# oadrian/GPUFluidSimulator

Measured on AMD Instinct MI355X. Metric: particle-steps/sec, higher is better.
Workload: dtype f32; 1 GPU; dam-break C3: 256x256x256 = 16777216 particles, grid 512^3, box 32.0, dt 5e-7, jittered lattice, FLOWING: timed after 6000 run-up steps on the device (+5 warm-up); particles=16777216, parallelism=1 GPU, whole domain, state=flow, runup_steps=6000

## Files before the change

gpufluidsimulator_amd/capi.py:

```python
from __future__ import annotations

import ctypes as C
import os

import numpy as np

HERE = os.path.dirname(os.path.abspath(__file__))
LIB_PATH = os.environ.get("SPH_HIP_LIB", os.path.join(HERE, "libsph_hip.so"))

PHASES = ("z-index", "sort", "b-grid", "dens", "force", "collision", "integrate")
HALO_RECORD_FLOATS = 8


class SphError(RuntimeError):
    pass


EXCHANGE_FN = C.CFUNCTYPE(C.c_int, C.c_void_p, C.c_int, C.c_void_p, C.c_size_t, C.c_void_p, C.c_size_t, C.c_void_p, C.c_size_t,
                          C.c_void_p, C.c_size_t, C.c_void_p)


class Transport(C.Structure):
    _fields_ = [("self", C.c_void_p), ("exchange", EXCHANGE_FN), ("host_buffers", C.c_int),
                ("abort", C.CFUNCTYPE(None, C.c_void_p))]
# ... 130 lines not shown
    "sph_slab_set_protocol": (C.c_int, [_P, C.c_int]),
    "sph_slab_protocol": (C.c_int, [_P, C.POINTER(C.c_uint64)]),
    "sph_destroy": (None, [_P]),
    "sph_set_stream": (C.c_int, [_P, _P]),
    "sph_set_params": (C.c_int, [_P, C.POINTER(Params)]),
    "sph_get_params": (C.c_int, [_P, C.POINTER(Params)]),
    "sph_sync": (C.c_int, [_P]),
    "sph_num_particles": (_U32, [_P]),
    "sph_capacity": (_U32, [_P]),
    "sph_upload": (C.c_int, [_P, _U32, _P, _P, _P]),
    "sph_set_by_index": (C.c_int, [_P, _U32, _U32, C.c_void_p, C.c_void_p]),
    "sph_reset_lattice": (C.c_int, [_P, C.POINTER(_U32), C.c_int, C.POINTER(C.c_float), C.c_uint64, _U32]),
    "sph_download": (C.c_int, [_P, _U32, _U32, _P, _P, _P, _P]),
    "sph_download_owned": (C.c_int, [_P, _P, _P, _P]),
    "sph_download_forces": (C.c_int, [_P, _U32, _U32, _P, _P, _P, _P]),
    "sph_snapshot_save": (C.c_int, [_P, C.c_char_p]),
    "sph_snapshot_load": (C.c_int, [_P, C.c_char_p]),
    "sph_snapshot_info": (C.c_int, [C.c_char_p, C.POINTER(_U32), C.POINTER(Params)]),
    "sph_set_colliders": (C.c_int, [_P, _U32, C.POINTER(Collider)]),
    "sph_get_colliders": (C.c_int, [_P, C.POINTER(_U32), C.POINTER(Collider)]),
    "sph_set_collider_bodies": (C.c_int, [_P, _U32, C.POINTER(ColliderBody)]),
    "sph_get_collider_impulses": (C.c_int, [_P, C.POINTER(_U32), C.POINTER(C.c_double), C.POINTER(C.c_uint64)]),
    "sph_emit": (C.c_int, [_P, _U32, _P, _P, _P, C.POINTER(_U32)]),
    "sph_remove": (C.c_int, [_P, _U32, C.POINTER(Region), C.POINTER(_U32), _P, _U32]),
    "sph_count_in_regions": (C.c_int, [_P, _U32, C.POINTER(Region), C.POINTER(_U32)]),
    "sph_camera_look_at": (C.c_int, [C.POINTER(Camera), _U32, _U32, C.POINTER(C.c_float), C.POINTER(C.c_float),
                                     C.POINTER(C.c_float), C.c_float, C.c_float, C.c_float]),
    "sph_render": (C.c_int, [_P, C.POINTER(Camera), C.POINTER(RenderStyle)]),
    "sph_render_read": (C.c_int, [_P, _P, _P, _P]),
    "sph_render_image_dev": (C.c_int, [_P, C.POINTER(_P), C.POINTER(_U32), C.POINTER(_U32)]),
    "sph_surface_defaults": (None, [C.POINTER(SurfaceStyle)]),
    "sph_render_surface": (C.c_int, [_P, C.POINTER(Camera), C.POINTER(RenderStyle), C.POINTER(SurfaceStyle)]),
    "sph_render_surface_read": (C.c_int, [_P, _P, _P, _P]),
    "sph_obstacle_lattice": (C.c_int, [_P, C.c_float, C.POINTER(C.c_float), C.POINTER(C.c_float), C.POINTER(ObstacleGrid)]),
    "sph_obstacle_build": (C.c_int, [_P, C.c_float, C.POINTER(C.c_float), C.POINTER(C.c_float), _U32, C.POINTER(Shape)]),
    "sph_obstacle_set_grid": (C.c_int, [_P, C.POINTER(ObstacleGrid), _P]),
    "sph_obstacle_clear": (C.c_int, [_P]),
    "sph_obstacle_set_motion": (C.c_int, [_P, C.POINTER(C.c_float), C.POINTER(C.c_float)]),
    "sph_obstacle_get": (C.c_int, [_P, C.POINTER(ObstacleGrid), C.POINTER(C.c_float), C.POINTER(C.c_float)]),
    "sph_obstacle_read": (C.c_int, [_P, _P]),
    "sph_obstacle_sample": (C.c_int, [_P, _U32, _P, _P, _P, _P]),
    "sph_obstacle_build_mesh": (C.c_int, [_P, C.POINTER(ObstacleMeshParams), C.POINTER(C.c_float), C.POINTER(C.c_float), _U32, _P,
                                          _U32, _P]),
    "sph_obstacle_build_mesh_dev": (C.c_int, [_P, C.POINTER(ObstacleMeshParams), C.POINTER(C.c_float), C.POINTER(C.c_float), _U32,
                                              _P, _U32, _P]),
    "sph_obstacle_build_obj": (C.c_int, [_P, C.POINTER(ObstacleMeshParams), C.POINTER(C.c_float), C.POINTER(C.c_float), C.c_char_p]),
    "sph_obstacle_mesh_stats": (C.c_int, [_P, C.POINTER(C.c_uint64)]),
    "sph_mesh_defaults": (None, [C.POINTER(MeshParams)]),
    "sph_mesh_lattice": (C.c_int, [_P, C.POINTER(MeshParams), C.POINTER(_U32), C.POINTER(C.c_float)]),
    "sph_mesh_extract": (C.c_int, [_P, C.POINTER(MeshParams), C.POINTER(_U32), C.POINTER(_U32)]),
    "sph_mesh_read": (C.c_int, [_P, _P, _P, _P]),
    "sph_mesh_dev": (C.c_int, [_P, C.POINTER(_P), C.POINTER(_P), C.POINTER(_P), C.POINTER(_U32), C.POINTER(_U32)]),
    "sph_mesh_save_obj": (C.c_int, [_P, C.c_char_p]),
    "sph_mesh_field_dims": (C.c_int, [_P, C.POINTER(_U32)]),
    "sph_mesh_field_read": (C.c_int, [_P, _P]),
    "sph_positions_dev": (C.c_int, [_P, C.POINTER(_P)]),
    "sph_download_positions4": (C.c_int, [_P, _P]),
    "sph_get_keys": (C.c_int, [_P, _P]),
    "sph_get_order": (C.c_int, [_P, _P]),
    "sph_get_cell_range": (C.c_int, [_P, _U32, C.POINTER(_U32), C.POINTER(_U32)]),
    "sph_get_cells": (C.c_int, [_P, _U32, _P, _P, _P]),
    "sph_cell_key": (_U32, [_P, _U32, _U32, _U32]),
    "sph_hash": (C.c_int, [_P]),
    "sph_sort": (C.c_int, [_P]),
    "sph_build_cells": (C.c_int, [_P]),
    "sph_density": (C.c_int, [_P]),
    "sph_force": (C.c_int, [_P]),
    "sph_collide": (C.c_int, [_P]),
    "sph_integrate": (C.c_int, [_P, C.c_float]),
    "sph_step": (C.c_int, [_P, C.c_float, _U32]),
    "sph_step_phased": (C.c_int, [_P, C.c_float, _U32]),
    "sph_force_collide_integrate": (C.c_int, [_P, C.c_float]),
    "sph_timing_enable": (C.c_int, [_P, C.c_int]),
    "sph_timing_get": (C.c_int, [_P, C.POINTER(C.c_float), C.POINTER(_U32)]),
    "sph_timing_reset": (C.c_int, [_P]),
    "sph_last_sort_skipped": (C.c_int, [_P]),
    "sph_sort_stats": (C.c_int, [_P, C.POINTER(C.c_uint64), C.POINTER(C.c_uint64), C.POINTER(C.c_uint64), C.POINTER(C.c_uint32),
                                 C.POINTER(C.c_uint64)]),
    "sph_set_sort_mode": (C.c_int, [_P, C.c_int]),
    "sph_set_direct_hull": (C.c_int, [_P, C.c_uint32]),
    "sph_set_pair_small_launch": (C.c_int, [_P, C.c_uint32]),
    "sph_set_block_order": (C.c_int, [_P, C.c_int, C.c_int, C.c_uint32]),
    "sph_sort_forms": (C.c_int, [_P, C.POINTER(C.c_uint64)]),
    "sph_test_trust_mover_hint": (C.c_int, [_P]),
    "sph_memory_stats": (None, [C.POINTER(C.c_uint64)]),
    "sph_test_fail_alloc": (None, [C.c_uint32]),
    "sph_test_guard": (None, [C.c_uint32, C.c_int]),
    "sph_test_guard_check": (C.c_int, [C.POINTER(C.c_uint64)]),
    "sph_test_scan": (C.c_int, [_P, C.c_int, C.c_uint32, C.c_void_p, C.c_void_p, C.c_void_p]),
    "sph_test_lower_bounds": (C.c_int, [_P, C.c_void_p, C.c_uint32, C.c_void_p, C.c_uint32, C.c_void_p]),
    "sph_set_precision": (C.c_int, [_P, C.c_int]),
    "sph_get_precision": (C.c_int, [_P]),
    "sph_migrants_count": (C.c_int, [_P, C.POINTER(_U32)]),
    "sph_slab_counts": (C.c_int, [_P, C.POINTER(_U32)]),
    "sph_migrants_pack": (C.c_int, [_P, C.POINTER(_P), _U32]),
    "sph_migrants_append": (C.c_int, [_P, _P, _U32]),
    "sph_halo_count": (C.c_int, [_P, C.POINTER(_U32)]),
    "sph_halo_pack": (C.c_int, [_P, C.POINTER(_P), _U32]),
    "sph_halo_pack_counts": (C.c_int, [_P, C.POINTER(_P), _U32, C.POINTER(_U32)]),
    "sph_halo_unpack": (C.c_int, [_P, _P, _U32, _P, _U32]),
    "sph_halo_pack_density": (C.c_int, [_P, C.POINTER(_P), _U32]),
    "sph_halo_unpack_density": (C.c_int, [_P, _P, _P]),
    "sph_layer_histogram": (C.c_int, [_P, _P, _U32]),
    "sph_rccl_unique_id": (C.c_int, [C.c_void_p]),
    "sph_rccl_transport_create": (C.c_int, [C.POINTER(C.POINTER(Transport)), C.c_void_p, C.c_int, C.c_int, C.c_int]),
    "sph_rccl_transport_destroy": (None, [C.POINTER(Transport)]),
    "sph_rccl_transport_selftest": (C.c_int, [C.POINTER(Transport), C.c_size_t]),
    "sph_rccl_transport_info": (C.c_int, [C.POINTER(Transport), C.POINTER(C.c_int)]),
    "sph_slab_ping": (C.c_int, [_P, C.c_size_t, _U32, C.POINTER(C.c_double)]),
    "sph_slab_recut": (C.c_int, [_P, _U32, _U32]),
    "sph_slab_recut_stats": (C.c_int, [_P, C.POINTER(C.c_uint64)]),
    "sph_slab_set_early_force": (C.c_int, [_P, C.c_int]),
    "sph_slab_early_force_stats": (C.c_int, [_P, C.POINTER(C.c_uint64)]),
    "sph_slab_timing_enable": (C.c_int, [_P, C.c_int]),
    "sph_slab_timing_reset": (C.c_int, [_P]),
    "sph_slab_timing_get": (C.c_int, [_P, C.POINTER(C.c_double)]),
    "sph_slab_test_raise_flag": (C.c_int, [_P, C.c_int]),
    "sph_slab_in_place_merges": (C.c_uint64, [C.c_void_p]),
    "sph_slab_exchanges": (C.c_uint64, [C.c_void_p]),
    "sph_slab_failed": (C.c_int, [C.c_void_p]),
    "sph_slab_create": (C.c_int, [C.POINTER(_P), _P, C.c_int, C.c_int, C.POINTER(Transport), _U32]),
    "sph_slab_destroy": (None, [_P]),
    "sph_slab_step": (C.c_int, [_P, C.c_float, _U32]),
    "sph_slab_sync": (C.c_int, [_P]),
    "sph_slab_stats": (C.c_int, [_P, C.POINTER(C.c_uint64)]),
    "sph_slab_counters": (C.c_int, [_P, C.POINTER(C.c_uint64)]),
    "sph_slab_set_wait_timeout": (C.c_int, [_P, C.c_double]),
    "sph_local_hub_create": (C.c_int, [C.POINTER(_P), C.c_int, C.c_int]),
    "sph_local_hub_destroy": (None, [_P]),
    "sph_local_hub_set_timeout": (C.c_int, [_P, C.c_double]),
    "sph_local_transport_create": (C.c_int, [C.POINTER(C.POINTER(Transport)), _P, C.c_int]),
    "sph_local_transport_destroy": (None, [C.POINTER(Transport)]),
    "sph_loop_transport_create": (C.c_int, [C.POINTER(C.POINTER(Transport)), C.c_float, C.c_double, C.c_double]),
    "sph_loop_transport_destroy": (None, [C.POINTER(Transport)]),
    "sph_ic_dam_break": (None, [C.POINTER(_U32), C.POINTER(C.c_float), C.c_int, C.c_uint64, C.c_uint64, _P, _P]),
    "sph_ic_random_box": (None, [C.c_uint64, C.POINTER(C.c_float), C.c_float, _U32, C.c_float, _P, _P]),
}

_lib = None
_torch_first = None


def load():
    global _lib, _torch_first
    if _lib is None:
        import sys
        _torch_first = "torch" in sys.modules
        if not os.path.exists(LIB_PATH):
            from . import build as _b
            _b.build()
        lib = C.CDLL(LIB_PATH)
        lenient = bool(os.environ.get("SPH_HIP_LIB_ALLOW_MISSING"))
        for name, (res, args) in SIGNATURES.items():
            if lenient and not hasattr(lib, name):
                continue
            fn = getattr(lib, name)
            fn.restype = res
            fn.argtypes = args
        if lib.sph_abi_version() != 2:
            raise SphError("libsph_hip.so ABI version mismatch")
        _lib = lib
    return _lib


def _check(rc):
    if rc < 0:
# ... 423 lines not shown

    def positions_dev(self):
        p = _P()
        _check(self.L.sph_positions_dev(self.h, C.byref(p)))
        return p.value

    def keys(self):
        out = np.empty(self.n, dtype=np.uint32)
        _check(self.L.sph_get_keys(self.h, out.ctypes.data))
        return out

    def order(self):
        out = np.empty(self.n, dtype=np.uint32)
        _check(self.L.sph_get_order(self.h, out.ctypes.data))
        return out

    def cells(self, max_cells=None):
        max_cells = self.n + 16 if max_cells is None else max_cells
        k = np.empty(max_cells, dtype=np.uint32)
        s = np.empty(max_cells, dtype=np.uint32)
        c = np.empty(max_cells, dtype=np.uint32)
        m = _check(self.L.sph_get_cells(self.h, max_cells, k.ctypes.data, s.ctypes.data, c.ctypes.data))
        m = min(m, max_cells)
        return k[:m], s[:m], c[:m]

    def cell_range(self, cell):
        a, b = _U32(), _U32()
        _check(self.L.sph_get_cell_range(self.h, int(cell), C.byref(a), C.byref(b)))
        return a.value, b.value

    def cell_key(self, x, y, z):
        return int(self.L.sph_cell_key(self.h, int(x), int(y), int(z)))

    def hash(self): _check(self.L.sph_hash(self.h))
    def sort(self): _check(self.L.sph_sort(self.h))
    def build_cells(self): _check(self.L.sph_build_cells(self.h))
    def density(self): _check(self.L.sph_density(self.h))
    def force(self): _check(self.L.sph_force(self.h))
    def collide(self): _check(self.L.sph_collide(self.h))
    def integrate(self, dt): _check(self.L.sph_integrate(self.h, float(dt)))
    def step(self, dt, n=1): _check(self.L.sph_step(self.h, float(dt), int(n)))
    def step_phased(self, dt, n=1): _check(self.L.sph_step_phased(self.h, float(dt), int(n)))
    def sync(self): _check(self.L.sph_sync(self.h))

    def timing(self, on=True): _check(self.L.sph_timing_enable(self.h, 1 if on else 0))
    def timing_reset(self): _check(self.L.sph_timing_reset(self.h))

    def sort_skipped(self):
        return bool(self.L.sph_last_sort_skipped(self.h))

    def sort_stats(self):
        a, b, k, m, t = C.c_uint64(), C.c_uint64(), C.c_uint64(), C.c_uint32(), C.c_uint64()
        _check(self.L.sph_sort_stats(self.h, C.byref(a), C.byref(b), C.byref(k), C.byref(m), C.byref(t)))
        return {"sorts": a.value, "merges": b.value, "skips": k.value, "last_movers": m.value, "movers_total": t.value}

    def set_precision(self, mixed_f16=False):
        _check(self.L.sph_set_precision(self.h, 1 if mixed_f16 else 0))

    def set_sort_mode(self, merge=True):
        _check(self.L.sph_set_sort_mode(self.h, int(merge)))

    def trust_mover_hint(self):
        _check(self.L.sph_test_trust_mover_hint(self.h))

    def test_scan(self, values):
        v = np.ascontiguousarray(values)
        assert v.ndim == 1 and v.dtype in (np.uint32, np.uint64), v.dtype
        out, total = np.empty_like(v), np.zeros(1, v.dtype)
        _check(self.L.sph_test_scan(self.h, 8 * v.dtype.itemsize, v.size, v.ctypes.data, out.ctypes.data, total.ctypes.data))
        return out, total[0]

    def test_lower_bounds(self, keys, targets):
        k, t = np.ascontiguousarray(keys), np.ascontiguousarray(targets)
        assert k.ndim == 1 and t.ndim == 1 and k.dtype == np.uint32 and t.dtype == np.uint32, (k.dtype, t.dtype)
        out = np.empty(t.size, np.uint32)
        _check(self.L.sph_test_lower_bounds(self.h, k.ctypes.data, k.size, t.ctypes.data, t.size, out.ctypes.data))
        return out

    def sort_forms(self):
        out = (C.c_uint64 * 3)()
        _check(self.L.sph_sort_forms(self.h, out))
        return tuple(int(v) for v in out)

    def set_block_order(self, xcd=True, ztile=True, strip_blocks_log2=4):
        _check(self.L.sph_set_block_order(self.h, int(bool(xcd)), int(bool(ztile)), int(strip_blocks_log2)))

    def set_direct_hull(self, slots=512):
        _check(self.L.sph_set_direct_hull(self.h, int(slots) & 0xFFFFFFFF))

    def set_pair_small_launch(self, slots):
        _check(self.L.sph_set_pair_small_launch(self.h, int(slots) & 0xFFFFFFFF))

    def timing_get(self):
        ms = (C.c_float * len(PHASES))()
        steps = _U32(0)
        _check(self.L.sph_timing_get(self.h, ms, C.byref(steps)))
        return {PHASES[k]: float(ms[k]) for k in range(len(PHASES))}, int(steps.value)

    def _pair(self, fn, *a):
        cnt = (_U32 * 2)()
        _check(fn(self.h, cnt, *a))
        return int(cnt[0]), int(cnt[1])

    def slab_counts(self):
        cnt = (_U32 * 4)()
        _check(self.L.sph_slab_counts(self.h, cnt))
        return tuple(int(v) for v in cnt)

    def force_collide_integrate(self, dt): _check(self.L.sph_force_collide_integrate(self.h, float(dt)))

    def migrants_count(self): return self._pair(self.L.sph_migrants_count)
    def halo_count(self): return self._pair(self.L.sph_halo_count)

    def migrants_pack(self, buf_lo, buf_hi, capacity):
        _check(self.L.sph_migrants_pack(self.h, (_P * 2)(buf_lo, buf_hi), int(capacity)))

    def migrants_append(self, buf, n):
        _check(self.L.sph_migrants_append(self.h, _P(buf), int(n)))

    def halo_pack(self, buf_lo, buf_hi, capacity, counts=None):
        if counts is None:
            _check(self.L.sph_halo_pack(self.h, (_P * 2)(buf_lo, buf_hi), int(capacity)))
        else:
            _check(self.L.sph_halo_pack_counts(self.h, (_P * 2)(buf_lo, buf_hi), int(capacity),
                                               (_U32 * 2)(int(counts[0]), int(counts[1]))))

    def halo_unpack(self, lo, n_lo, hi, n_hi):
        _check(self.L.sph_halo_unpack(self.h, _P(lo), int(n_lo), _P(hi), int(n_hi)))

    def halo_pack_density(self, buf_lo, buf_hi, capacity):
        _check(self.L.sph_halo_pack_density(self.h, (_P * 2)(buf_lo, buf_hi), int(capacity)))

    def halo_unpack_density(self, lo, hi):
        _check(self.L.sph_halo_unpack_density(self.h, _P(lo), _P(hi)))

    def layer_histogram(self):
        n = int(self.params.grid[2])
        out = np.zeros(n, dtype=np.uint32)
        _check(self.L.sph_layer_histogram(self.h, out.ctypes.data, n))
        return out
```

gpufluidsimulator_amd/csrc/sph_capi.hip:

```cpp
#include "sph_device.hpp"

#include <cmath>
#include <cstdarg>
#include <cstdlib>
#include <cstring>
#include <mutex>
#include <new>
#include <vector>

namespace sph {

template <class T>
__global__ __launch_bounds__(1024) void k_test_scan(const T* __restrict__ in, uint32_t n, T* __restrict__ out, T* __restrict__ total) {
    __shared__ T lds[1024 / 64];
    const T sum = scan_array_one_block<1024>(n, lds, [&](uint32_t i) { return in[i]; }, [&](uint32_t i, T before) { out[i] = before; });
    if (threadIdx.x == 0) *total = sum;
}

template <class T>
static int test_scan(sph_ctx* c, Buffers& mem, uint32_t n, const void* in, void* out, void* total) {
    T *d_in = nullptr, *d_out = nullptr, *d_total = nullptr;
    int rc;
    if ((rc = mem.alloc(&d_in, n, false)) || (rc = mem.alloc(&d_out, n, false)) || (rc = mem.alloc(&d_total, 1, false))) return rc;
    if (n) SPH_HIP(hipMemcpyAsync(d_in, in, (size_t)n * sizeof(T), hipMemcpyHostToDevice, c->stream));
// ... 171 lines not shown
    ph.gas_constant = p->gas_constant;
    const float poly6 = 315.f / (65.f * PI_F * powf(p->h, 9.f));
    const float spiky = 45.f / (PI_F * powf(p->h, 6.f));
    ph.poly6_mass = p->mass * poly6;
    ph.spiky_half_mass = p->mass * spiky * 0.5f;
    const float visc = p->viscosity != 0.f ? p->viscosity : 1.f;
    ph.visc_coef = (visc * p->mass) * spiky;
    ph.cp_scale = ph.spiky_half_mass / ph.visc_coef;
    ph.visc_on = p->viscosity != 0.f ? 1.f : 0.f;
    ph.gravity_y = p->gravity_y;
    ph.wall_eps = p->wall_eps;
    ph.wall_damping = p->wall_damping;
    const double cd = (double)p->collision_param * 2.0 * (double)p->particle_radius;
    float r2max = (float)(cd * cd);
    for (int k = 0; k < 8; k++) r2max = nextafterf(r2max, INFINITY);
    while ((double)sqrtf(r2max) > cd) r2max = nextafterf(r2max, 0.f);
    ph.coll_dist2 = r2max;
    ph.coll_mass = p->mass * (1.f + p->restitution);
    for (int a = 0; a < 3; a++) { ph.box_min[a] = p->box_min[a]; ph.box_max[a] = p->box_max[a]; }
    return SPH_OK;
}

static int create_impl(sph_ctx** out, int device, uint32_t capacity, const sph_params* p, uint32_t z_lo, uint32_t z_hi,
                       uint32_t gcap, bool slab, uint32_t ghost_layers = 1) {
    SPH_REQUIRE(out && p, SPH_E_INVALID, "null argument");
    *out = nullptr;
    SPH_REQUIRE(capacity > 0 && (uint64_t)capacity + 2ull * gcap < (1ull << 31), SPH_E_INVALID, "bad capacity");
    int ndev = 0;
    hipError_t e = hipGetDeviceCount(&ndev);
    if (e != hipSuccess || ndev <= 0) {
        set_error("no HIP device available (%s): libsph_hip has no CPU fallback", hipGetErrorString(e));
        return SPH_E_DEVICE;
    }
    if (device < 0) device = g_device;
    SPH_REQUIRE(device < ndev, SPH_E_DEVICE, "device %d out of range (%d devices)", device, ndev);
    SPH_HIP(hipSetDevice(device));
    hipDeviceProp_t prop;
    SPH_HIP(hipGetDeviceProperties(&prop, device));
    if (strncmp(prop.gcnArchName, "gfx950", 6) != 0) {
        set_error("device %d is %s; libsph_hip is built for gfx950 (MI355X) only", device, prop.gcnArchName);
        return SPH_E_DEVICE;
    }
    sph_ctx* c = new (std::nothrow) sph_ctx();
    SPH_REQUIRE(c, SPH_E_NOMEM, "out of host memory");
    c->device = device;
    c->ghost_layers = slab ? ghost_layers : 1u;
    int rc = derive(c, p, z_lo, z_hi, slab);
    if (rc) { delete c; return rc; }
    c->cap = capacity; c->gcap = gcap; c->tot = capacity + 2 * gcap; c->slab = slab;
    c->own_off = gcap;
    c->pos_out_cap = slab ? 0 : capacity;
    Buffers& m = c->mem;
    const size_t tot = (size_t)c->tot + 256;
    rc = m.alloc(&c->posi, tot, true);
    if (!rc) rc = m.alloc(&c->velr, tot, true);
    if (!rc) rc = m.alloc(&c->posi2, tot, true);
    if (!rc) rc = m.alloc(&c->velr2, tot, true);
    if (!rc) rc = m.alloc(&c->keyS, tot, true);
    if (!rc) rc = m.alloc(&c->keyS2, tot, true);
    if (!rc) rc = m.alloc(&c->dp, tot, true);
    if (!rc) rc = m.alloc(&c->cw, tot, true);
    if (!rc) rc = m.alloc(&c->fpress, tot, false);
    if (!rc) rc = m.alloc(&c->fvisc, tot, false);
    if (!rc) rc = m.alloc(&c->dvel, tot, false);
    if (!rc) rc = m.alloc(&c->pos_out, (size_t)c->pos_out_cap, false);
    if (!rc) rc = m.alloc(&c->table.base, (size_t)c->grid.ncells + 2, true);
    if (!rc) table_init(c, c->table.base, c->grid.ncells);
    if (!rc) rc = sort_buffers_alloc(c);
    if (const char* env = getenv("SPH_BLOCK_ORDER")) {
        int x = 1, z = 1, sh = 4, zd = 1, xr = 1;
        if (sscanf(env, "%d,%d,%d,%d,%d", &x, &z, &sh, &zd, &xr) >= 1) {
            c->order_xcd = x != 0; c->order_ztile = z != 0; if (sh >= 1 && sh <= 10) c->order_strip_sh = (uint32_t)sh;
            c->order_ztile_dens = zd != 0; c->order_xrot = xr != 0;
        }
    }
    if (const char* env = getenv("SPH_PAIR_SMALL_SLOTS")) {
        unsigned long v = 0;
        if (sscanf(env, "%lu", &v) == 1) c->pair_small_slots = v > 0xFFFFFFFFul ? 0xFFFFFFFFu : (uint32_t)v;
    }
    if (const char* env = getenv("SPH_PAIR_CLAMP")) {
        int v = 1;
        if (sscanf(env, "%d", &v) == 1) c->pair_clamp = v != 0;
    }
    if (rc) { m.free_all(); delete c; return rc; }
    *out = c;
    return SPH_OK;
}

void timing_collect(sph_ctx* c) {
    for (size_t k = 0; k + 3 <= c->events.size(); k += 3) {
        hipEvent_t a = c->events[k], b = c->events[k + 1];
        int phase = (int)(intptr_t)c->events[k + 2];
        hipEventSynchronize(b);
        float ms = 0.f;
        if (hipEventElapsedTime(&ms, a, b) == hipSuccess) c->ph_ms[phase] += ms;
        hipEventDestroy(a);
        hipEventDestroy(b);
    }
    c->events.clear();
}

int step_hash(sph_ctx* c, bool ghosts_to_sort) {
    PhaseTimer t(c, SPH_PH_ZINDEX);
    const SlotRange live = live_slots(c);
    int rc = c->sort_merge && c->order_valid && table_covers(c, live.lo, live.hi) ? table_leave_to_sort(c, ghosts_to_sort)
                                                                                 : launch_cells_clear(c);
    if (rc) return rc;
    rc = launch_hash(c);
    if (rc) return rc;
    c->keys_fresh = false;
    c->stage = sph_ctx::ST_HASHED;
    return SPH_OK;
}

int step_sort(sph_ctx* c, bool* owned_build_pending) {
    PhaseTimer t(c, SPH_PH_SORT);
    int rc = launch_sort(c, owned_build_pending);
    if (rc) return rc;
    c->n_glo = c->n_ghi = 0;
    c->halo_n_valid = false;
    c->stage = sph_ctx::ST_SORTED;
    results_stale(c);
    return SPH_OK;
}

int step_cells(sph_ctx* c) {
    PhaseTimer t(c, SPH_PH_BGRID);
    const SlotRange live = live_slots(c);
    if (!table_covers(c, live.lo, live.hi)) {
        int rc = launch_cells_build(c);
        if (rc) return rc;
    }
    c->stage = sph_ctx::ST_CELLS;
    return SPH_OK;
}

static int do_density(sph_ctx* c) {
    PhaseTimer t(c, SPH_PH_DENS);
    int rc = launch_density(c);
    if (rc) return rc;
    c->have_dens = true;
    return SPH_OK;
}

}

namespace sph {
int set_slab_range(sph_ctx* c, uint32_t z_lo, uint32_t z_hi) {
    SPH_REQUIRE(c && c->slab, SPH_E_INVALID, "set_slab_range needs a slab context");
    sph_ctx tmp;
    tmp.params = c->params;
    tmp.ghost_layers = c->ghost_layers;
    int rc = derive(&tmp, &c->params, z_lo, z_hi, true);
    if (rc) return rc;
    if (tmp.grid.ncells > c->table.alloc) {
        SPH_HIP(hipStreamSynchronize(c->stream));
        uint2* base = nullptr;
        rc = c->mem.alloc(&base, (size_t)tmp.grid.ncells + 2, true);
        if (rc) return rc;
        c->mem.release(&c->table.base);
        table_init(c, base, tmp.grid.ncells);
    }
    c->grid = tmp.grid; c->z_lo = z_lo; c->z_hi = z_hi; c->key_bits = tmp.key_bits;
    table_forget(c);
    order_lost(c);
    results_stale(c);
    c->n_glo = c->n_ghi = 0;
    c->halo_n_valid = false;
    return SPH_OK;
}
}

using namespace sph;

__global__ __launch_bounds__(256) void k_set_by_index(float4* __restrict__ posi, float4* __restrict__ velr, uint32_t n,
                                                      uint32_t first, uint32_t count, const float* __restrict__ pos,
                                                      const float* __restrict__ vel, float4* __restrict__ pos_by_index) {
    const uint32_t i = blockIdx.x * 256u + threadIdx.x;
    if (i >= n) return;
    float4 p = posi[i];
    const uint32_t k = __float_as_uint(p.w) - first;
    if (k >= count) return;
    if (pos) {
        p.x = pos[3 * k]; p.y = pos[3 * k + 1]; p.z = pos[3 * k + 2];
        posi[i] = p;
        if (pos_by_index) pos_by_index[first + k] = make_float4(p.x, p.y, p.z, 1.0f);
    }
    if (vel) velr[i] = make_float4(vel[3 * k], vel[3 * k + 1], vel[3 * k + 2], 0.f);
}


__global__ __launch_bounds__(256) void k_gather_cells(const uint32_t* __restrict__ keys, uint32_t m,
                                                      const uint2* __restrict__ cells, uint2* __restrict__ out) {
    const uint32_t k = blockIdx.x * 256u + threadIdx.x;
    if (k < m) out[k] = cells[keys[k]];
}

static inline uint32_t idx_of(const float4& p) { uint32_t u; memcpy(&u, &p.w, 4); return u; }

static int install_records(sph_ctx* c, uint32_t n, const float4* hp, const float4* hv) {
// ... 542 lines not shown
        }
        tmp.free_all();
        if (rc) return rc;
        for (uint32_t k = 0; k < take; k++) {
            if (key) key[k] = uniq[k];
            if (start) start[k] = got[k].x - lo;
            if (count) count[k] = got[k].y - got[k].x;
        }
    }
    return (int)m;
}

uint32_t sph_cell_key(const sph_ctx* c, uint32_t x, uint32_t y, uint32_t z) {
    if (!c) return 0;
    return ((uint32_t)((int32_t)z - c->grid.z_off) * c->grid.g[1] + y) * c->grid.g[0] + x;
}

int sph_hash(sph_ctx* c) {
    SPH_REQUIRE(c, SPH_E_INVALID, "null context");
    SPH_HIP(hipSetDevice(c->device));
    return step_hash(c);
}

int sph_sort(sph_ctx* c) {
    SPH_REQUIRE(c, SPH_E_INVALID, "null context");
    SPH_REQUIRE(c->stage == sph_ctx::ST_HASHED, SPH_E_STATE, "sph_sort needs sph_hash first");
    SPH_HIP(hipSetDevice(c->device));
    return step_sort(c);
}

int sph_build_cells(sph_ctx* c) {
    SPH_REQUIRE(c, SPH_E_INVALID, "null context");
    SPH_REQUIRE(c->stage >= sph_ctx::ST_SORTED, SPH_E_STATE, "sph_build_cells needs sph_sort first");
    SPH_HIP(hipSetDevice(c->device));
    return step_cells(c);
}

int sph_density(sph_ctx* c) {
    SPH_REQUIRE(c, SPH_E_INVALID, "null context");
    SPH_REQUIRE(c->stage >= sph_ctx::ST_CELLS && c->table.valid, SPH_E_STATE, "sph_density needs sph_build_cells first");
    SPH_HIP(hipSetDevice(c->device));
    return do_density(c);
}

int sph_force(sph_ctx* c) {
    SPH_REQUIRE(c, SPH_E_INVALID, "null context");
    SPH_REQUIRE(c->stage >= sph_ctx::ST_CELLS && c->have_dens, SPH_E_STATE, "sph_force needs sph_density first");
    SPH_HIP(hipSetDevice(c->device));
    PhaseTimer t(c, SPH_PH_FORCE);
    int rc = launch_force(c, true, false, false, 0.f);
    if (rc) return rc;
    c->have_force = true;
    return SPH_OK;
}

int sph_collide(sph_ctx* c) {
    SPH_REQUIRE(c, SPH_E_INVALID, "null context");
    SPH_REQUIRE(c->stage >= sph_ctx::ST_CELLS && c->table.valid, SPH_E_STATE, "sph_collide needs sph_build_cells first");
    SPH_HIP(hipSetDevice(c->device));
    PhaseTimer t(c, SPH_PH_COLLISION);
    int rc = launch_force(c, false, true, false, 0.f);
    if (rc) return rc;
    c->have_coll = true;
    return SPH_OK;
}

int sph_integrate(sph_ctx* c, float dt) {
    SPH_REQUIRE(c, SPH_E_INVALID, "null context");
    SPH_REQUIRE(c->have_dens && c->have_force && c->have_coll, SPH_E_STATE,
                "sph_integrate needs sph_density, sph_force and sph_collide first");
    SPH_HIP(hipSetDevice(c->device));
    PhaseTimer t(c, SPH_PH_INTEGRATE);
    int rc = launch_integrate(c, dt);
    if (rc) return rc;
    c->have_force = c->have_coll = false;
    return SPH_OK;
}

int sph_step(sph_ctx* c, float dt, uint32_t n_steps) {
    SPH_REQUIRE(c, SPH_E_INVALID, "null context");
    SPH_HIP(hipSetDevice(c->device));
    for (uint32_t s = 0; s < n_steps; s++) {
        int rc = step_hash(c);
        if (!rc) rc = step_sort(c);
        if (!rc) rc = step_cells(c);
        if (!rc) rc = do_density(c);
        if (rc) return rc;
        {
            PhaseTimer t(c, SPH_PH_FORCE);
            rc = launch_force(c, true, true, true, dt);
            if (rc) return rc;
        }
        c->have_force = c->have_coll = false;
        if (c->timing) { c->timed_steps++; if (c->events.size() > 3 * 4096) timing_collect(c); }
    }
    return SPH_OK;
}

int sph_force_collide_integrate(sph_ctx* c, float dt) {
    SPH_REQUIRE(c, SPH_E_INVALID, "null context");
    SPH_REQUIRE(c->stage >= sph_ctx::ST_CELLS && c->have_dens, SPH_E_STATE,
                "sph_force_collide_integrate needs sph_density first");
    SPH_HIP(hipSetDevice(c->device));
    PhaseTimer t(c, SPH_PH_FORCE);
    int rc = launch_force(c, true, true, true, dt);
    if (rc) return rc;
    c->have_force = c->have_coll = false;
    return SPH_OK;
}

int sph_step_phased(sph_ctx* c, float dt, uint32_t n_steps) {
    for (uint32_t s = 0; s < n_steps; s++) {
        int rc = sph_hash(c);
        if (!rc) rc = sph_sort(c);
        if (!rc) rc = sph_build_cells(c);
        if (!rc) rc = sph_density(c);
        if (!rc) rc = sph_force(c);
        if (!rc) rc = sph_collide(c);
        if (!rc) rc = sph_integrate(c, dt);
        if (rc) return rc;
        if (c->timing) { c->timed_steps++; if (c->events.size() > 3 * 4096) timing_collect(c); }
    }
    return SPH_OK;
}

int sph_timing_enable(sph_ctx* c, int on) {
    SPH_REQUIRE(c, SPH_E_INVALID, "null context");
    c->timing = on != 0;
    return SPH_OK;
}

int sph_timing_get(sph_ctx* c, float ms[SPH_PH_COUNT], uint32_t* n_steps) {
    SPH_REQUIRE(c && ms, SPH_E_INVALID, "null argument");
    SPH_HIP(hipSetDevice(c->device));
    timing_collect(c);
    for (int k = 0; k < SPH_PH_COUNT; k++) ms[k] = (float)c->ph_ms[k];
    if (n_steps) *n_steps = c->timed_steps;
    return SPH_OK;
}

int sph_timing_reset(sph_ctx* c) {
    SPH_REQUIRE(c, SPH_E_INVALID, "null context");
    SPH_HIP(hipSetDevice(c->device));
    timing_collect(c);
    for (int k = 0; k < SPH_PH_COUNT; k++) c->ph_ms[k] = 0;
    c->timed_steps = 0;
    return SPH_OK;
}

int sph_last_sort_skipped(const sph_ctx* c) { return c && c->last_sort_skipped ? 1 : 0; }

int sph_set_precision(sph_ctx* c, int precision) {
    SPH_REQUIRE(c, SPH_E_INVALID, "null context");
    SPH_REQUIRE(precision == SPH_PRECISION_F32 || precision == SPH_PRECISION_MIXED_F16, SPH_E_INVALID,
                "unknown precision %d", precision);
    c->precision = precision;
    return SPH_OK;
}

int sph_get_precision(const sph_ctx* c) { return c ? c->precision : SPH_PRECISION_F32; }

int sph_set_sort_mode(sph_ctx* c, int merge) {
    SPH_REQUIRE(c, SPH_E_INVALID, "null context");
    c->sort_merge = merge != 0;
    c->sort_merge_always = merge == 2;
    return SPH_OK;
}

int sph_test_trust_mover_hint(sph_ctx* c) {
    SPH_REQUIRE(c, SPH_E_INVALID, "null context");
    c->sort_form_both_until = 0;
    return SPH_OK;
}

int sph_sort_forms(const sph_ctx* c, uint64_t out[3]) {
    SPH_REQUIRE(c && out, SPH_E_INVALID, "null argument");
    for (int k = 0; k < 3; k++) out[k] = c->sort_forms[k];
    return SPH_OK;
}

int sph_set_block_order(sph_ctx* c, int xcd, int ztile, uint32_t strip_blocks_log2) {
    SPH_REQUIRE(c, SPH_E_INVALID, "null context");
    SPH_REQUIRE(strip_blocks_log2 >= 1u && strip_blocks_log2 <= 10u, SPH_E_INVALID, "strip of 2^%u blocks", strip_blocks_log2);
    c->order_xcd = xcd != 0;
    c->order_ztile = c->order_ztile_dens = ztile != 0;
    c->order_strip_sh = strip_blocks_log2;
    return SPH_OK;
}

int sph_set_direct_hull(sph_ctx* c, uint32_t slots) {
    SPH_REQUIRE(c, SPH_E_INVALID, "null context");
    c->direct_hull = slots;
    return SPH_OK;
}

int sph_set_pair_small_launch(sph_ctx* c, uint32_t slots) {
    SPH_REQUIRE(c, SPH_E_INVALID, "null context");
    c->pair_small_slots = slots;
    return SPH_OK;
}

int sph_sort_stats(sph_ctx* c, uint64_t* sorts, uint64_t* merges, uint64_t* skips, uint32_t* last_movers,
                   uint64_t* movers_total) {
    SPH_REQUIRE(c, SPH_E_INVALID, "null context");
    SPH_HIP(hipSetDevice(c->device));
    SPH_HIP(hipStreamSynchronize(c->stream));
    if (movers_total) {
        unsigned long long t = 0;
        SPH_HIP(hipMemcpy(&t, c->mm_total, sizeof(t), hipMemcpyDeviceToHost));
        *movers_total = t;
    }
    if (sorts) *sorts = c->sort_calls;
    if (merges) *merges = c->sort_merges;
    if (skips) *skips = c->sort_skips;
    if (last_movers) *last_movers = c->mm_count_host[HW_MOVERS];
    return SPH_OK;
}

void sph_memory_stats(uint64_t out[3]) {
    if (out) for (int k = 0; k < 3; k++) out[k] = g_mem_stats[k].load();
}

void sph_test_fail_alloc(uint32_t k) { g_fail_alloc.store(k); }

void sph_test_guard(uint32_t band_bytes, int fill_unzeroed) {
    if (band_bytes % 4096u) { set_error("guard bands of %u bytes: not a multiple of 4096", band_bytes); return; }
    g_guard_fill.store(band_bytes && fill_unzeroed ? 1u : 0u);
    g_guard_band.store(band_bytes);
}

int sph_test_guard_check(uint64_t out[4]) {
    SPH_REQUIRE(out, SPH_E_INVALID, "null argument");
    return guard_check_all(out);
}

int sph_test_scan(sph_ctx* c, int bits, uint32_t n, const void* in, void* out, void* total) {
    SPH_REQUIRE(c && total && (n == 0 || (in && out)), SPH_E_INVALID, "null argument");
    SPH_REQUIRE(bits == 32 || bits == 64, SPH_E_INVALID, "a scan of %d-bit values", bits);
    SPH_HIP(hipSetDevice(c->device));
    Buffers mem;
    const int rc = bits == 32 ? test_scan<uint32_t>(c, mem, n, in, out, total) : test_scan<uint64_t>(c, mem, n, in, out, total);
    mem.free_all();
    return rc;
}

int sph_test_lower_bounds(sph_ctx* c, const uint32_t* keys, uint32_t n, const uint32_t* targets, uint32_t m, uint32_t* out) {
    SPH_REQUIRE(c && (n == 0 || keys) && (m == 0 || (targets && out)), SPH_E_INVALID, "null argument");
    SPH_REQUIRE(m <= LB_MAX, SPH_E_INVALID, "%u targets: at most %u", m, LB_MAX);
    SPH_HIP(hipSetDevice(c->device));
    LbTargets tg{{}, m};
    for (uint32_t k = 0; k < m; k++) tg.v[k] = targets[k];
    Buffers mem;
    const int rc = test_lower_bounds(c, mem, keys, n, tg, out);
    mem.free_all();
    return rc;
}

}
```

gpufluidsimulator_amd/csrc/sph_common.hpp:

```cpp
#pragma once

#include <hip/hip_runtime.h>

#include <atomic>
#include <cstdint>
#include <cstdio>
#include <cstring>
#include <string>
#include <utility>
#include <vector>

#include "../../include/sph_hip.h"

namespace sph {

constexpr int WAVE = 64;
#ifndef SPH_SORT_KPT
#define SPH_SORT_KPT 16
#endif
constexpr uint32_t SORT_TILE_KEYS = 256 * SPH_SORT_KPT;
#ifndef SPH_PAIR_SMALL_SLOTS_DEFAULT
#define SPH_PAIR_SMALL_SLOTS_DEFAULT 524288u
#endif
constexpr uint32_t MM_TILE_CHUNKS = 256;
// ... 63 lines not shown
    Buffers(const Buffers&) = delete;
    Buffers& operator=(const Buffers&) = delete;
    template <class T> int alloc(T** p, size_t count, bool zero) {
        const size_t bytes = (count ? count : 1) * sizeof(T);
        int rc = take((void**)p, bytes, false, false, !zero);
        if (rc || !zero || hipMemset((void*)*p, 0, bytes) == hipSuccess) return rc;
        release(p);
        set_error("hipMemset of %zu bytes failed", bytes);
        return SPH_E_DEVICE;
    }
    template <class T> int alloc_host(T** p, size_t count, T** dev_view = nullptr) {
        int rc = take((void**)p, count * sizeof(T), true, dev_view != nullptr, true);
        if (rc || !dev_view || hipHostGetDevicePointer((void**)dev_view, (void*)*p, 0) == hipSuccess) return rc;
        release(p);
        set_error("hipHostGetDevicePointer failed");
        return SPH_E_NOMEM;
    }
    template <class T> void release(T** p) {
        for (size_t k = live.size(); k-- > 0;)
            if (live[k].p == (void*)*p) { drop(live[k]); live.erase(live.begin() + k); break; }
        *p = nullptr;
    }
    void free_all() {
        while (!live.empty()) { drop(live.back()); live.pop_back(); }
    }

private:
    int take(void** p, size_t bytes, bool pinned, bool mapped, bool unzeroed) {
        const char* fn = !pinned ? "hipMalloc" : mapped ? "hipHostMalloc(mapped)" : "hipHostMalloc";
        *p = nullptr;
        uint32_t k = g_fail_alloc.load();
        while (k && !g_fail_alloc.compare_exchange_weak(k, k - 1)) {}
        const uint32_t band = g_guard_band.load();
        const size_t total = band ? ((bytes + 3) & ~(size_t)3) + 2 * (size_t)band : bytes;
        const hipError_t e = k == 1 ? hipErrorOutOfMemory
                           : pinned ? hipHostMalloc(p, total, mapped ? hipHostMallocMapped : hipHostMallocDefault) : hipMalloc(p, total);
        if (e != hipSuccess) {
            *p = nullptr;
            set_error("%s of %zu bytes failed: %s", fn, bytes, hipGetErrorString(e));
            return SPH_E_NOMEM;
        }
        if (band) {
            if (guard_adopt(*p, bytes, band, pinned, unzeroed && g_guard_fill.load())) {
                if (pinned) hipHostFree(*p); else hipFree(*p);
                *p = nullptr;
                set_error("the guard bands of %zu bytes could not be written", bytes);
                return SPH_E_DEVICE;
            }
            *p = (char*)*p + band;
        }
        live.push_back(Rec{*p, bytes, pinned, band});
        g_mem_stats[pinned] += bytes; g_mem_stats[2] += 1;
        return SPH_OK;
    }
    static void drop(const Rec& r) {
        void* base = r.p;
        if (r.band) { guard_retire(r.p, r.bytes, r.band, r.pinned); base = (char*)r.p - r.band; }
        if (r.pinned) hipHostFree(base); else hipFree(base);
        g_mem_stats[r.pinned] -= r.bytes; g_mem_stats[2] -= 1;
    }
};

enum class TableLeft : uint8_t {
    NOTHING,
    OWNED,
    OWNED_AND_GHOSTS
};

struct CellTable {
    uint2* cells = nullptr;
    uint2* base = nullptr;
    uint32_t alloc = 0;
    uint32_t lo = 0, hi = 0;
    bool valid = false;
    TableLeft left = TableLeft::NOTHING;
};

struct MoverMarks {
    bool marked = false;
    bool scanned = false;
    uint32_t off = 0, n = 0;
    uint32_t scan_seq = 0;
    bool counted_valid = false;
};

enum HostWord : uint32_t {
    HW_MOVERS = 0,
    HW_FIRST_KEY,
    HW_LAST_KEY,
    HW_BUILD_SEQ,
    HW_COUNT_SEQ,
    HW_WORDS = 8
};

}

struct sph_ctx {
    int device = 0;
    hipStream_t stream = nullptr;
    sph::Buffers mem;
    sph_params params{};
    int precision = SPH_PRECISION_F32;
    sph::GridDesc grid{};
    sph::Phys phys{};

    uint32_t cap = 0;
    uint32_t gcap = 0;
    uint32_t tot = 0;
    bool slab = false;
    uint32_t z_lo = 0, z_hi = 0;
    uint32_t ghost_layers = 1;

    uint32_t n = 0;
    uint32_t own_off = 0;
    uint32_t n_glo = 0, n_ghi = 0;
    uint32_t halo_n[2] = {0, 0};
    bool halo_n_valid = false;

    float4* posi = nullptr;
    float4* velr = nullptr;
    float4* posi2 = nullptr;
    float4* velr2 = nullptr;
    uint32_t* keyS = nullptr;
    uint32_t* keyS2 = nullptr;
    float2* dp = nullptr;
    float2* cw = nullptr;
    float4* fpress = nullptr;
    float4* fvisc = nullptr;
    float4* dvel = nullptr;
    float4* pos_out = nullptr;
    uint32_t pos_out_cap = 0;
    uint32_t next_index = 0;

    uint32_t n_colliders = 0;
    sph_collider colliders[SPH_MAX_COLLIDERS] = {};
    bool tracked = false;
    sph::SphereBodies bodies{};
    sph::Spheres* trk_table = nullptr;
    double* trk_partial = nullptr;
    uint32_t* trk_mask = nullptr;
    double* trk_J = nullptr;

    sph_obstacle_grid ob_grid{};
    float* ob_phi = nullptr;
    float* ob_brick = nullptr;
    float ob_off[3] = {0.f, 0.f, 0.f}, ob_vel[3] = {0.f, 0.f, 0.f};
    uint64_t* ob_mesh_work = nullptr;
    uint32_t* ob_mesh_marks = nullptr;

    uint64_t* rd_keys = nullptr;
    uint32_t* rd_rgba = nullptr;
    uint32_t* rd_id = nullptr;
    float* rd_depth = nullptr;
    uint32_t rd_alloc_w = 0, rd_alloc_h = 0;
    uint32_t rd_w = 0, rd_h = 0;
    bool rd_valid = false;
    unsigned long long* rd_counts = nullptr;
    float* rd_sf_raw = nullptr;
    float* rd_sf_pong = nullptr;
    uint32_t* rd_sf_thick = nullptr;
    float* rd_sf_normal = nullptr;
    bool rd_surface = false;
    bool rd_sf_thick_on = false;

    uint32_t* mesh_field = nullptr;
    uint32_t* mesh_vbase = nullptr;
    uint32_t* mesh_aux = nullptr;
    float* mesh_vpos = nullptr;
    float* mesh_vnrm = nullptr;
    uint32_t* mesh_tri = nullptr;
    uint32_t mesh_nodes_cap = 0, mesh_v_cap = 0, mesh_t_cap = 0;
    uint32_t mesh_dims[3] = {0, 0, 0};
    uint32_t mesh_nv = 0, mesh_nt = 0;
    bool mesh_valid = false;

    uint32_t direct_hull = 512;
    uint32_t pair_small_slots = SPH_PAIR_SMALL_SLOTS_DEFAULT;
    bool pair_clamp = true;
    bool order_xcd = true, order_ztile = true;
    bool order_ztile_dens = true, order_xrot = true;
    uint32_t order_strip_sh = 4;

    sph::CellTable table;
    bool keys_fresh = false;

    uint32_t* k0 = nullptr; uint32_t* v0 = nullptr;
    uint32_t* k1 = nullptr; uint32_t* v1 = nullptr;
    uint32_t* os_hist = nullptr;
    uint32_t* os_base = nullptr;
    uint32_t* os_tickets = nullptr;
    uint32_t* os_tot = nullptr;
    uint32_t os_groups_cap = 0;
    unsigned long long* os_status = nullptr;
    uint32_t* os_status32 = nullptr;
    uint32_t os_epoch = 0;
    uint32_t* os_err_host = nullptr;
    uint32_t* os_err_dev = nullptr;
    uint32_t sort_blocks_cap = 0;
    uint32_t key_bits = 0;
    const uint32_t* last_perm = nullptr;
    bool keep_perm = false;
    bool sort_merge = true;
    bool sort_merge_always = false;
    bool order_valid = false;
    bool last_sort_skipped = false;
    bool host_paced = false;
    uint32_t sort_seq_issued = 0;
    uint64_t sort_merges = 0, sort_calls = 0, sort_skips = 0;
    uint64_t sort_form_both_until = 0;
    uint64_t sort_forms[3] = {0, 0, 0};
    uint64_t* mm_mask = nullptr;
    uint32_t* mm_M64 = nullptr;
    uint32_t* mm_tile_cnt = nullptr; uint32_t* mm_tile_off = nullptr;
    uint32_t* mm_k0 = nullptr; uint32_t* mm_k1 = nullptr; uint32_t* mm_v1 = nullptr;
    uint32_t* mm_count = nullptr;
    uint32_t* mm_count_host = nullptr;
    uint32_t* mm_count_host_dev = nullptr;
    unsigned long long* mm_total = nullptr;
    sph::MoverMarks marks;
    uint32_t* mm_tileL = nullptr;
    uint32_t* mm_tileA = nullptr;
    uint32_t* d_scratch = nullptr;
    uint32_t* h_scratch = nullptr;

    enum Stage { ST_LOADED = 0, ST_HASHED, ST_SORTED, ST_CELLS } stage = ST_LOADED;
    bool have_force = false, have_coll = false, have_dens = false;

    bool timing = false;
    std::vector<hipEvent_t> events;
    double ph_ms[SPH_PH_COUNT] = {0};
    uint32_t timed_steps = 0;
};

namespace sph {

void mm_set_marks(sph_ctx* c);
void mm_scan_marks(sph_ctx* c);
void mm_drop_marks(sph_ctx* c, bool counted = false);
int hip_fail(hipError_t e, const char* what, const char* file, int line);

#define SPH_HIP(call)                                                        \
    do {                                                                     \
        hipError_t e__ = (call);                                             \
        if (e__ != hipSuccess) return sph::hip_fail(e__, #call, __FILE__, __LINE__); \
    } while (0)

#define SPH_REQUIRE(cond, code, ...)          \
    do {                                      \
        if (!(cond)) {                        \
            sph::set_error(__VA_ARGS__);      \
            return (code);                    \
        }                                     \
    } while (0)

int launch_hash(sph_ctx* c);
int launch_reset_lattice(sph_ctx* c, const uint32_t lattice[3], int jitter, const float jitter_dims[3], uint64_t start,
                         uint32_t count);
int launch_sort(sph_ctx* c, bool* owned_build_pending = nullptr);
int launch_merge_arrivals(sph_ctx* c, uint32_t n_in, uint32_t n_front = 0);
int launch_cells_clear(sph_ctx* c);
void table_forget(sph_ctx* c);
int table_drop_ends(sph_ctx* c, uint32_t m_lo, uint32_t m_hi);
int table_drop_ghosts(sph_ctx* c);
int table_leave_to_sort(sph_ctx* c, bool ghosts_too);
TableLeft table_take_left(sph_ctx* c);
int launch_cells_clear_range(sph_ctx* c, uint32_t lo, uint32_t hi);
int launch_cells_build_range(sph_ctx* c, uint32_t lo, uint32_t hi, uint32_t seq = 0);
int launch_cells_clear_2ranges(sph_ctx* c, uint32_t lo0, uint32_t hi0, uint32_t lo1, uint32_t hi1);
int launch_cells_build_2ranges(sph_ctx* c, uint32_t lo0, uint32_t hi0, uint32_t lo1, uint32_t hi1);
int launch_cells_build(sph_ctx* c);
constexpr uint32_t CELLS_SPT = 4;
inline uint32_t cells_build_blocks(uint32_t count) { return (count + 256u * CELLS_SPT - 1u) / (256u * CELLS_SPT); }
int launch_density(sph_ctx* c);
int launch_force(sph_ctx* c, bool force, bool collide, bool integrate, float dt);
int launch_density_range(sph_ctx* c, uint32_t lo, uint32_t hi);
int launch_density_hole(sph_ctx* c, uint32_t lo, uint32_t hi, uint32_t hole_lo, uint32_t hole_hi);
int launch_density_dev_range(sph_ctx* c, const uint32_t* range_dev, uint32_t max_count);
int launch_force_dev_range(sph_ctx* c, const uint32_t* range_dev, uint32_t max_count, float dt);
int launch_force_hole(sph_ctx* c, uint32_t lo, uint32_t hi, uint32_t hole_lo, uint32_t hole_hi, bool force, bool collide,
                      bool integrate, float dt, bool mark);
bool force_begin(sph_ctx* c, bool integrate);
int launch_force_range(sph_ctx* c, uint32_t lo, uint32_t hi, bool force, bool collide, bool integrate, float dt, bool mark);
int force_finish(sph_ctx* c, bool integrate, bool mark, float dt);
int set_slab_range(sph_ctx* c, uint32_t z_lo, uint32_t z_hi);
int step_hash(sph_ctx* c, bool ghosts_to_sort = false);
int step_sort(sph_ctx* c, bool* owned_build_pending = nullptr);
int step_cells(sph_ctx* c);
int launch_integrate(sph_ctx* c, float dt);
inline bool have_obstacle(const sph_ctx* c) { return c->ob_phi != nullptr; }
int launch_obstacle_push(sph_ctx* c, bool fused, bool mark);
void advance_obstacle(sph_ctx* c, float dt);
int obstacle_ctx(const sph_ctx* c, const char* who);
int lattice_resolve(const sph_ctx* c, float spacing, const float* lo, const float* hi, sph_obstacle_grid* G);
float ob_clamp_distance(const sph_obstacle_grid& G);
int install_begin(sph_ctx* c, const sph_obstacle_grid& G);
int install_finish(sph_ctx* c);
void release_obstacle(sph_ctx* c);
int launch_spheres_install(sph_ctx* c);
int launch_spheres_radii(sph_ctx* c);
struct RecSide { float4* rec; float4* posi; float4* velr; uint32_t* key; uint32_t n; };
int launch_pack_records(hipStream_t st, const RecSide& lo, const RecSide& hi);
int launch_unpack_records(hipStream_t st, const RecSide& lo, const RecSide& hi, const GridDesc& g, uint32_t G, volatile uint32_t* err_word);
int launch_unpack_dp(hipStream_t st, const float2* src_lo, float2* dp_lo, float2* cw_lo, uint32_t n_lo, const float2* src_hi, float2* dp_hi,
                     float2* cw_hi, uint32_t n_hi, const Phys& ph);
constexpr uint32_t LB_MAX = 32;
struct LbTargets { uint32_t v[LB_MAX]; uint32_t m; };
int launch_lower_bounds(hipStream_t st, const uint32_t* keys, uint32_t n, const LbTargets& tg, uint32_t* out, volatile uint32_t* out_host);
enum Bound {
    B_OWN_BEGIN, B_FIRST_END,
    B_LAST_BEGIN, B_OWN_END,
    B_DEEP_LO, B_DEEP_HI,
    B_NEAR_LO, B_NEAR_HI,
    B_EARLY_LO, B_EARLY_HI,
    B_LAYER5,
    B_COUNT
};
__host__ __device__ inline uint32_t bound_layer(uint32_t b, uint32_t G, uint32_t zl) {
    const uint32_t d0 = min(G + 3u, zl - 1u), d1 = zl >= 2u * G + 6u ? zl - G - 3u : d0;
    const uint32_t e0 = min(G + 2u, zl - 1u), e1 = zl >= 2u * G + 4u ? zl - G - 2u : e0;
    const uint32_t f0 = min(G + 5u, zl - 1u), f1 = zl >= 2u * G + 11u ? zl - G - 5u : f0;
    const uint32_t d_end = max(d1, d0), e_end = max(e1, e0), f_end = max(f1, f0), layer5 = min(G + 4u, zl - 1u);
    const uint32_t z[B_COUNT] = {G, G + 1u, zl - G - 1u, zl - G,
                                 d0, d_end, e0, e_end,
                                 f0, f_end, layer5};
    return z[b];
}
inline LbTargets layer_bound_targets(const sph_ctx* c) {
    const uint32_t layer = c->grid.g[0] * c->grid.g[1], G = c->ghost_layers, zl = c->grid.zl;
    return LbTargets{{bound_layer(B_OWN_BEGIN, G, zl) * layer, bound_layer(B_FIRST_END, G, zl) * layer,
                      bound_layer(B_LAST_BEGIN, G, zl) * layer, bound_layer(B_OWN_END, G, zl) * layer}, 4u};
}
int launch_headers(hipStream_t st, float4* out_lo, float4* out_hi, float4 lo, float4 hi);
int sort_buffers_alloc(sph_ctx* c);
int tracked_buffers_alloc(sph_ctx* c);

inline uint32_t ceil_div(uint32_t a, uint32_t b) { return (a + b - 1) / b; }

inline void results_stale(sph_ctx* c) { c->have_dens = c->have_force = c->have_coll = false; }
inline void mover_count_unknown(sph_ctx* c) { c->sort_form_both_until = c->sort_calls + 5; }
inline void positions_moved(sph_ctx* c) { c->keys_fresh = false; c->stage = sph_ctx::ST_LOADED; }
inline void order_lost(sph_ctx* c) { positions_moved(c); c->order_valid = false; }
inline void swap_state(sph_ctx* c, bool keys) {
    std::swap(c->posi, c->posi2);
    std::swap(c->velr, c->velr2);
    if (keys) { std::swap(c->keyS, c->keyS2); c->own_off = c->gcap; }
}
inline bool table_covers(const sph_ctx* c, uint32_t lo, uint32_t hi) { return c->table.valid && c->table.lo == lo && c->table.hi == hi; }
inline void table_init(sph_ctx* c, uint2* base, uint32_t alloc) { c->table.base = base; c->table.cells = base + 1; c->table.alloc = alloc; }
inline void table_set(sph_ctx* c, uint32_t lo, uint32_t hi) { c->table.lo = lo; c->table.hi = hi; c->table.valid = true; }
struct SlotRange { uint32_t lo, hi; };
inline SlotRange live_slots(const sph_ctx* c) { return SlotRange{c->own_off - c->n_glo, c->own_off + c->n + c->n_ghi}; }

inline void pack_records(uint32_t n, const float* pos, const float* vel, const uint32_t* index, uint32_t first, float4* hp, float4* hv) {
    for (size_t i = 0; i < n; i++) {
        const uint32_t idx = index ? index[i] : first + (uint32_t)i;
        float w;
        memcpy(&w, &idx, 4);
        hp[i] = make_float4(pos[3 * i], pos[3 * i + 1], pos[3 * i + 2], w);
        hv[i] = vel ? make_float4(vel[3 * i], vel[3 * i + 1], vel[3 * i + 2], 0.f) : make_float4(0.f, 0.f, 0.f, 0.f);
    }
}

struct PhaseTimer {
    sph_ctx* c; int phase; hipEvent_t a = nullptr, b = nullptr;
    PhaseTimer(sph_ctx* c_, int ph) : c(c_), phase(ph) {
        if (!c->timing) return;
        if (hipEventCreate(&a) != hipSuccess || hipEventCreate(&b) != hipSuccess) { a = b = nullptr; return; }
        hipEventRecord(a, c->stream);
    }
// ... 12 lines not shown
```

gpufluidsimulator_amd/csrc/sph_pairs.hip:

```cpp
#include "sph_device.hpp"

namespace sph {

#ifndef SPH_PAIR_THREADS
#define SPH_PAIR_THREADS 256
#endif
constexpr int PAIR_THREADS = SPH_PAIR_THREADS;
constexpr int PAIR_WAVES = PAIR_THREADS / WAVE;
#ifndef SPH_DENS_THREADS
#define SPH_DENS_THREADS SPH_PAIR_THREADS
#endif
constexpr int DENS_THREADS = SPH_DENS_THREADS;
constexpr int SMALL_THREADS_PAIR = 128;
static inline bool small_blocks(const sph_ctx* c) { return c->n < c->pair_small_slots; }
static inline bool pair_clamp(const sph_ctx* c) { return c->pair_clamp && c->phys.h <= 1.f && c->phys.h2 <= 1.f; }
constexpr int PIECE = 128;

typedef float v2f __attribute__((ext_vector_type(2)));
typedef const volatile __attribute__((address_space(3))) v2f* lds_v2f_ptr;
typedef const volatile __attribute__((address_space(3))) float* lds_f32_ptr;
typedef const volatile __attribute__((address_space(3))) char* lds_byte_ptr;

__global__ __launch_bounds__(256) void k_cells_clear(const uint32_t* __restrict__ key, uint32_t lo, uint32_t hi,
                                                     uint2* __restrict__ cells) {
    uint32_t s = lo + blockIdx.x * 256u + threadIdx.x;
    if (s >= hi) return;
    uint32_t k = key[s];
    if (s == lo || key[s - 1] != k) cells[k] = make_uint2(0u, 0u);
}

__global__ __launch_bounds__(256) void k_cells_build(const uint32_t* __restrict__ key, uint32_t lo, uint32_t hi,
                                                     uint2* __restrict__ cells, volatile uint32_t* __restrict__ ends_host, uint32_t seq) {
    cells_build_thread(key, lo, hi, cells, ends_host, seq, blockIdx.x * 256u + threadIdx.x);
}

__global__ __launch_bounds__(256) void k_cells_clear2(const uint32_t* __restrict__ key, uint32_t lo0, uint32_t hi0,
                                                      uint32_t lo1, uint32_t hi1, uint2* __restrict__ cells) {
    const uint32_t t = blockIdx.x * 256u + threadIdx.x, n0 = hi0 - lo0;
    const uint32_t lo = t < n0 ? lo0 : lo1, hi = t < n0 ? hi0 : hi1;
    const uint32_t s = t < n0 ? lo0 + t : lo1 + (t - n0);
    if (s >= hi) return;
    const uint32_t k = key[s];
    if (s == lo || key[s - 1] != k) cells[k] = make_uint2(0u, 0u);
}

__global__ __launch_bounds__(256) void k_cells_build2(const uint32_t* __restrict__ key, uint32_t lo0, uint32_t hi0,
                                                      uint32_t lo1, uint32_t hi1, uint2* __restrict__ cells) {
    const uint32_t t = blockIdx.x * 256u + threadIdx.x, n0 = hi0 - lo0;
    const uint32_t lo = t < n0 ? lo0 : lo1, hi = t < n0 ? hi0 : hi1;
    const uint32_t s = t < n0 ? lo0 + t : lo1 + (t - n0);
    if (s >= hi) return;
    const uint32_t k = key[s];
    if (s == lo || key[s - 1] != k) cells[k].x = s;
    if (s + 1 == hi || key[s + 1] != k) cells[k].y = s + 1;
}

int launch_cells_clear_2ranges(sph_ctx* c, uint32_t lo0, uint32_t hi0, uint32_t lo1, uint32_t hi1) {
    if (hi0 < lo0) hi0 = lo0;
    if (hi1 < lo1) hi1 = lo1;
    const uint32_t tot = (hi0 - lo0) + (hi1 - lo1);
    if (!tot) return SPH_OK;
    hipLaunchKernelGGL(k_cells_clear2, dim3(ceil_div(tot, 256)), dim3(256), 0, c->stream, c->keyS, lo0, hi0, lo1, hi1, c->table.cells);
    SPH_HIP(hipGetLastError());
    return SPH_OK;
}

int launch_cells_build_2ranges(sph_ctx* c, uint32_t lo0, uint32_t hi0, uint32_t lo1, uint32_t hi1) {
    if (hi0 < lo0) hi0 = lo0;
    if (hi1 < lo1) hi1 = lo1;
    const uint32_t tot = (hi0 - lo0) + (hi1 - lo1);
    if (!tot) return SPH_OK;
    hipLaunchKernelGGL(k_cells_build2, dim3(ceil_div(tot, 256)), dim3(256), 0, c->stream, c->keyS, lo0, hi0, lo1, hi1, c->table.cells);
    SPH_HIP(hipGetLastError());
    return SPH_OK;
}

void table_forget(sph_ctx* c) { c->table.valid = false; c->table.left = TableLeft::NOTHING; }

int launch_cells_clear(sph_ctx* c) {
    const CellTable& t = c->table;
    if (t.valid && t.hi > t.lo) {
        hipLaunchKernelGGL(k_cells_clear, dim3(ceil_div(t.hi - t.lo, 256)), dim3(256), 0, c->stream, c->keyS, t.lo, t.hi, t.cells);
        SPH_HIP(hipGetLastError());
// ... 46 lines not shown
    SPH_HIP(hipGetLastError());
    return SPH_OK;
}

int launch_cells_build(sph_ctx* c) {
    const SlotRange live = live_slots(c);
    int rc;
    if (table_covers(c, c->own_off, c->own_off + c->n)) {
        rc = launch_cells_build_2ranges(c, live.lo, c->own_off, c->own_off + c->n, live.hi);
    } else {
        rc = launch_cells_clear(c);
        if (!rc) rc = launch_cells_build_range(c, live.lo, live.hi);
    }
    if (rc) return rc;
    table_set(c, live.lo, live.hi);
    return SPH_OK;
}

struct Rows {
    uint32_t lo[9], hi[9];
};

__device__ __forceinline__ void lane_rows(const uint2* __restrict__ cells, const GridDesc& g, uint32_t key, bool active,
                                          Rows& R) {
    const uint32_t gx = g.g[0], gy = g.g[1];
    uint32_t cx, cy, lz;
    if (((gx & (gx - 1u)) | (gy & (gy - 1u))) == 0u) {
        const uint32_t sx = 31u - (uint32_t)__clz((int)gx), sy = 31u - (uint32_t)__clz((int)gy);
        cx = key & (gx - 1u);
        cy = (key >> sx) & (gy - 1u);
        lz = key >> (sx + sy);
    } else {
        cx = key % gx;
        const uint32_t t = key / gx;
        cy = t % gy;
        lz = t / gy;
    }
    const bool has_l = cx > 0u, has_r = cx + 1u < gx;
    const bool y_ok[3] = {cy > 0u, true, cy + 1u < gy};
    const bool z_ok[3] = {lz > 0u, true, lz + 1u < g.zl};
    const int sy_ = (int)gx, sz_ = (int)(gx * gy);
    uint2 a[9], b[9], d[9];
    bool ok[9];
#pragma unroll
    for (int dz = -1; dz <= 1; dz++) {
#pragma unroll
        for (int dy = -1; dy <= 1; dy++) {
            const int r = (dz + 1) * 3 + (dy + 1);
            ok[r] = active && y_ok[dy + 1] && z_ok[dz + 1];
            const uint2* p = cells + (ok[r] ? (int)key + dz * sz_ + dy * sy_ : (int)key);
            a[r] = p[-1]; b[r] = p[0]; d[r] = p[1];
        }
    }
#pragma unroll
    for (int r = 0; r < 9; r++) {
        const bool na = ok[r] && has_l && a[r].y > a[r].x, nb = ok[r] && b[r].y > b[r].x,
                   nd = ok[r] && has_r && d[r].y > d[r].x;
        R.lo[r] = na ? a[r].x : (nb ? b[r].x : (nd ? d[r].x : 0u));
        R.hi[r] = nd ? d[r].y : (nb ? b[r].y : (na ? a[r].y : 0u));
    }
}

__device__ __forceinline__ void lane_row_one(const uint2* __restrict__ cells, const GridDesc& g, uint32_t key, bool active,
                                             int dz, int dy, uint32_t& lo, uint32_t& hi) {
    const uint32_t gx = g.g[0], gy = g.g[1];
    uint32_t cx, cy, lz;
    if (((gx & (gx - 1u)) | (gy & (gy - 1u))) == 0u) {
        const uint32_t sx = 31u - (uint32_t)__clz((int)gx), sy = 31u - (uint32_t)__clz((int)gy);
        cx = key & (gx - 1u); cy = (key >> sx) & (gy - 1u); lz = key >> (sx + sy);
    } else {
        cx = key % gx;
        const uint32_t t = key / gx;
        cy = t % gy; lz = t / gy;
    }
    const bool ok = active && (int)cy + dy >= 0 && (int)cy + dy < (int)gy && (int)lz + dz >= 0 && (int)lz + dz < (int)g.zl;
    const uint2* p = cells + (ok ? (int)key + dz * (int)(gx * gy) + dy * (int)gx : (int)key);
    const uint2 a = p[-1], b = p[0], d = p[1];
    const bool na = ok && cx > 0u && a.y > a.x, nb = ok && b.y > b.x, nd = ok && cx + 1u < gx && d.y > d.x;
    lo = na ? a.x : (nb ? b.x : (nd ? d.x : 0u));
    hi = nd ? d.y : (nb ? b.y : (na ? a.y : 0u));
}

#ifndef SPH_DENS_OCC
#define SPH_DENS_OCC 6
#endif
#ifndef SPH_FORCE_OCC
#define SPH_FORCE_OCC 5
#endif

__device__ __forceinline__ float in_vgpr(float x) {
    asm volatile("" : "+v"(x));
    return x;
}

__device__ __forceinline__ float inv_sqrt(float x) { return __builtin_amdgcn_rsqf(x); }

template <bool CLAMP>
__device__ __forceinline__ float cut_below_zero(float x) {
    if constexpr (CLAMP) return __builtin_amdgcn_fmed3f(x, 0.f, 1.f);
    else return fmaxf(x, 0.f);
}

__device__ __forceinline__ void wave_lds_sync() {
    __builtin_amdgcn_fence(__ATOMIC_RELEASE, "wavefront");
    __builtin_amdgcn_wave_barrier();
    __builtin_amdgcn_fence(__ATOMIC_ACQUIRE, "wavefront");
}

constexpr int lds_ent(int threads) { return (threads / WAVE + 1) * PIECE + 8; }
#ifndef SPH_DENS_UNROLL
#define SPH_DENS_UNROLL 4
#endif
constexpr int UNROLL = SPH_DENS_UNROLL;
#ifndef SPH_FORCE_UNROLL
#define SPH_FORCE_UNROLL 2
#endif
#ifndef SPH_EXACT_DIV
#define SPH_EXACT_DIV 0
#endif

struct Hulls {
    uint32_t A[9], B[9];
};

__device__ __forceinline__ void wave_hulls(const Rows& R, Hulls& H) {
#pragma unroll
    for (int r = 0; r < 9; r++) {
        const uint64_t m = __ballot(R.hi[r] > R.lo[r]);
        if (m == 0ull) { H.A[r] = 0u; H.B[r] = 0u; continue; }
        const int first = __builtin_ctzll(m), last = 63 - __builtin_clzll(m);
        H.A[r] = (uint32_t)__builtin_amdgcn_readlane((int)R.lo[r], first);
        H.B[r] = (uint32_t)__builtin_amdgcn_readlane((int)R.hi[r], last);
    }
}

template <class Load, class Store, class Work>
__device__ __forceinline__ void traverse(const Hulls& H, Load&& load, Store&& store, Work&& work) {
    auto first_behind = [&](int r, uint32_t& a) {
        bool any = false;
#pragma unroll
        for (int q = 8; q > r; q--) {
            uint32_t end = H.B[q];
            asm volatile("" : "+s"(end));
            if (end != 0u) { a = H.A[q]; any = true; }
        }
        return any;
    };
    uint32_t a_next = 0u;
    if (!first_behind(-1, a_next)) return;
    load(a_next);
#pragma unroll
    for (int r = 0; r < 9; r++) {
        if (H.A[r] >= H.B[r]) continue;
        for (uint32_t a = H.A[r]; a < H.B[r]; a += PIECE) {
            store();
            bool more = true;
            a_next = a + PIECE;
            if (a_next >= H.B[r]) more = first_behind(r, a_next);
            if (more) load(a_next);
            wave_lds_sync();
            work(r, a, min(a + PIECE, H.B[r]));
            wave_lds_sync();
        }
    }
}

__device__ __forceinline__ bool wave_has_long_hull(const Hulls& H, uint32_t key, uint32_t direct_hull) {
    const uint32_t k0 = (uint32_t)__builtin_amdgcn_readlane((int)key, 0), k1 = (uint32_t)__builtin_amdgcn_readlane((int)key, 63);
    if (k1 - k0 <= 64u && direct_hull >= 128u) return false;
    bool any = false;
#pragma unroll
    for (int r = 0; r < 9; r++) any = any || (H.B[r] > H.A[r] && H.B[r] - H.A[r] > direct_hull);
    return any;
}

template <class Row>
__device__ __forceinline__ void direct_rows(const uint2* __restrict__ cells, const GridDesc& g, uint32_t key, bool active,
                                            Row&& row) {
#pragma clang loop unroll(disable)
    for (int r = 0; r < 9; r++) {
        uint32_t l0, l1;
        lane_row_one(cells, g, key, active, r / 3 - 1, r % 3 - 1, l0, l1);
        const uint32_t len = l1 > l0 ? l1 - l0 : 0u;
        const uint32_t T = wave_max_u32(len);
        if (T) row(l0, len, T);
    }
}

struct Targets {
    uint32_t lo, hi, gap_lo, gap_len;
    const uint32_t* dev;
    uint32_t direct_hull;
    BlockOrder order;
};

__device__ __forceinline__ uint32_t pair_block() {
    const uint32_t rot = max(gridDim.x >> 6, 1u);
    return blockIdx.x < rot ? gridDim.x - rot + blockIdx.x : blockIdx.x - rot;
}

__device__ __forceinline__ bool wave_targets(const Targets& T, uint32_t wave, uint32_t lane, uint32_t& i, uint32_t& hi,
                                             uint32_t& first) {
    uint32_t lo = T.lo;
    hi = T.hi;
    if (T.dev) { lo = T.dev[0]; hi = T.dev[1]; }
    first = lo + (ordered_block(pair_block(), gridDim.x, T.order) * (blockDim.x >> 6) + wave) * WAVE;
    if (first >= T.gap_lo) first += T.gap_len;
    i = first + lane;
    return first < hi;
}

#ifdef SPH_PAIR_STATS
__device__ unsigned long long g_pair_stats[12];
__device__ int g_pair_stats_on;
#define PAIR_STAT(k, v) do { if (lane == 0 && g_pair_stats_on) atomicAdd(&g_pair_stats[k], (unsigned long long)(v)); } while (0)
extern "C" void sph_debug_pair_stats(unsigned long long* out, int on) {
    (void)hipDeviceSynchronize();
    (void)hipMemcpyFromSymbol(out, HIP_SYMBOL(g_pair_stats), sizeof(g_pair_stats));
    unsigned long long z[12] = {};
    (void)hipMemcpyToSymbol(HIP_SYMBOL(g_pair_stats), z, sizeof(z));
    (void)hipMemcpyToSymbol(HIP_SYMBOL(g_pair_stats_on), &on, sizeof(on));
}
#else
#define PAIR_STAT(k, v) do { } while (0)
#endif

template <int THREADS, bool CLAMP>
__global__ __launch_bounds__(THREADS, SPH_DENS_OCC) void k_density(const float4* __restrict__ posi,
                                                                   const uint32_t* __restrict__ keyS,
                                                                   const uint2* __restrict__ cells,
                                                                   float2* __restrict__ dp, float2* __restrict__ cw,
                                                                   Targets tg, GridDesc g, Phys ph) {
    static_assert(UNROLL % 2 == 0, "the z-pair walk reads candidates two at a time");
    constexpr int DENS_ENT = lds_ent(THREADS);
    __shared__ float2 s_xy[DENS_ENT];
    __shared__ __attribute__((aligned(8))) float s_z[DENS_ENT];
    __shared__ __attribute__((aligned(8))) float s_zo_[DENS_ENT + 2];
    float* const s_zo = s_zo_ + 2;
    if (tg.dev && tg.dev[0] + ordered_block(pair_block(), gridDim.x, tg.order) * (uint32_t)THREADS >= tg.dev[1]) return;
    for (uint32_t k = threadIdx.x; k < DENS_ENT; k += THREADS) {
        s_xy[k] = make_float2(0.f, 0.f);
        s_z[k] = 0.f;
        s_zo_[k] = 0.f;
        if (k < 2u) s_zo_[DENS_ENT + k] = 0.f;
    }
    __syncthreads();
    const uint32_t wave = threadIdx.x >> 6, lane = threadIdx.x & 63u;
    const uint32_t slice = wave * PIECE;
    uint32_t i, tgt_hi, wave_first;
    if (!wave_targets(tg, wave, lane, i, tgt_hi, wave_first)) return;
    const bool active = i < tgt_hi;
    const uint32_t ii = active ? i : tgt_hi - 1;
    const float4 pi = posi[ii];
    Rows R;
    const uint32_t my_key = keyS[ii];
    lane_rows(cells, g, my_key, active, R);
    Hulls H;
    wave_hulls(R, H);
    float4 q0, q1;
    const uint32_t lane16 = lane << 4;
    float acc = 0.f;
    const float h2_v = in_vgpr(ph.h2);
    auto pair_math = [&](float x, float y, float z, bool valid) {
        const float dx = pi.x - x, dy = pi.y - y, dz = pi.z - z;
        float d = cut_below_zero<CLAMP>(fmaf(-dz, dz, fmaf(-dy, dy, fmaf(-dx, dx, h2_v))));
        d = valid ? d : 0.f;
        acc = fmaf(d * d, d, acc);
    };
    auto finish = [&]() {
        if (active) {
            float rho = acc * ph.poly6_mass;
            float p = fmaxf(0.f, ph.gas_constant * (rho - ph.rest_density));
            dp[i] = make_float2(rho, p);
            cw[i] = neighbour_terms(ph, rho, p);
        }
    };
    if (wave_has_long_hull(H, my_key, tg.direct_hull)) {
        const uint32_t me = active ? i : tgt_hi - 1u;
        direct_rows(cells, g, keyS[me], active, [&](uint32_t l0, uint32_t len, uint32_t T) {
            for (uint32_t t = 0; t < T; t += 2u) {
                float4 q[2];
#pragma unroll
                for (uint32_t u = 0; u < 2u; u++) q[u] = posi[t + u < len ? l0 + t + u : me];
#pragma unroll
                for (uint32_t u = 0; u < 2u; u++) pair_math(q[u].x, q[u].y, q[u].z, t + u < len);
            }
        });
        finish();
        return;
    }
    traverse(
        H,
        [&](uint32_t a) {
            const float4* const pa = posi + a;
            q0 = lane_elem(pa, lane16);
            q1 = lane_elem(pa + WAVE, lane16);
        },
        [&]() {
            s_xy[slice + lane] = make_float2(q0.x, q0.y);
            s_z[slice + lane] = q0.z;
            s_xy[slice + WAVE + lane] = make_float2(q1.x, q1.y);
            s_z[slice + WAVE + lane] = q1.z;
            s_zo[(int)(slice + lane) - 1] = q0.z;
            s_zo[slice + WAVE + lane - 1u] = q1.z;
        },
        [&](int r, uint32_t a, uint32_t b) {
            const uint32_t l0 = max(R.lo[r], a), l1 = min(R.hi[r], b);
            const uint32_t len = l1 > l0 ? l1 - l0 : 0u;
            const uint32_t rel = len ? l0 - a : 0u;
            uint32_t idx = slice + rel;
            const uint32_t tmin = wave_min_u32_uniform_first(len) & ~(uint32_t)(UNROLL - 1);
            lds_v2f_ptr zp = (lds_v2f_ptr)(((rel & 1u) ? (const float*)s_zo - 1 : (const float*)s_z) + idx);
            auto group = [&](uint32_t t, bool check) {
#pragma unroll
                for (int u = 0; u < UNROLL; u += 2) {
                    const v2f xy0 = ((lds_v2f_ptr)s_xy)[idx + u], xy1 = ((lds_v2f_ptr)s_xy)[idx + u + 1];
                    const v2f zz = zp[u >> 1];
                    pair_math(xy0.x, xy0.y, zz.x, !check || t + u < len);
                    pair_math(xy1.x, xy1.y, zz.y, !check || t + u + 1 < len);
                }
                idx += UNROLL;
                zp += UNROLL / 2;
            };
            uint32_t t = 0;
            for (; t < tmin; t += UNROLL) group(t, false);
#ifdef SPH_PAIR_STATS
            const uint32_t stat_t0 = t;
#endif
            for (; __ballot(t < len) != 0ull; t += UNROLL) group(t, true);
            PAIR_STAT(11, t - stat_t0);
        });
    finish();
}
// ... 739 lines not shown
                           c->trk_mask, ceil_div(c->n, 64u), c->trk_J, c->bodies, dt, c->phys);
        SPH_HIP(hipGetLastError());
        return SPH_OK;
    }
    for (uint32_t j = 0; j < c->n_colliders; j++)
        for (int a = 0; a < 3; a++) c->colliders[j].center[a] = c->colliders[j].center[a] + dt * c->colliders[j].velocity[a];
    return SPH_OK;
}

int launch_force_hole(sph_ctx* c, uint32_t lo, uint32_t hi, uint32_t hole_lo, uint32_t hole_hi, bool force, bool collide,
                      bool integrate, float dt, bool mark) {
    if (hi <= lo) return SPH_OK;
    SPH_REQUIRE(((lo - c->own_off) & 63u) == 0u, SPH_E_INVALID, "force sub-range does not start on a 64-slot chunk");
    uint32_t threads;
    Targets tg = targets_with_hole(lo, hi, hole_lo, hole_hi, threads);
    tg.direct_hull = c->direct_hull;
    const bool small = small_blocks(c);
    const uint32_t bt = small ? (uint32_t)SMALL_THREADS_PAIR : (uint32_t)PAIR_THREADS;
    tg.order = block_order(c, ceil_div(threads, bt), integrate && force);
    SPH_REQUIRE(tg.gap_len == 0u || (((tg.gap_lo - lo) | tg.gap_len) & 63u) == 0u || tg.gap_lo + tg.gap_len == hi, SPH_E_INVALID,
                "force hole is not made of whole 64-slot chunks");
    if (threads == 0) return SPH_OK;
    if (force && !collide && !integrate) force_kernel<true, false, false>(c, small, tg, threads, dt, mark, false);
    else if (!force && collide && !integrate) force_kernel<false, true, false>(c, small, tg, threads, dt, mark, false);
    else if (force && collide && integrate) {
        if (c->tracked) force_kernel<true, true, true>(c, small, tg, threads, dt, mark, false, tracked_pack(c));
        else if (c->n_colliders) force_kernel<true, true, true>(c, small, tg, threads, dt, mark, false, sphere_table(c));
        else force_kernel<true, true, true>(c, small, tg, threads, dt, mark, false);
    } else {
        set_error("launch_force: unsupported combination");
        return SPH_E_INVALID;
    }
    SPH_HIP(hipGetLastError());
    return SPH_OK;
}

int launch_force_dev_range(sph_ctx* c, const uint32_t* range_dev, uint32_t max_count, float dt) {
    if (max_count == 0) return SPH_OK;
    const Targets tg{0u, 0u, 0xFFFFFFFFu, 0u, range_dev, c->direct_hull, BlockOrder{0u, 0u, 0u, 0u, 0u}};
    if (c->n_colliders) force_kernel<true, true, true>(c, small_blocks(c), tg, max_count, dt, false, true, sphere_table(c));
    else force_kernel<true, true, true>(c, small_blocks(c), tg, max_count, dt, false, true);
    SPH_HIP(hipGetLastError());
    return SPH_OK;
}

int launch_force_range(sph_ctx* c, uint32_t lo, uint32_t hi, bool force, bool collide, bool integrate, float dt, bool mark) {
    return launch_force_hole(c, lo, hi, hi, hi, force, collide, integrate, dt, mark);
}

bool force_begin(sph_ctx* c, bool integrate) {
    if (integrate) mm_drop_marks(c);
    return integrate && c->sort_merge && c->order_valid;
}

int force_finish(sph_ctx* c, bool integrate, bool mark, float dt) {
    if (!integrate) return SPH_OK;
    const int rc = advance_colliders(c, dt);
    swap_state(c, false);
    c->keys_fresh = true;
    if (mark) {
        mm_set_marks(c);
        mm_scan_marks(c);
    }
    return rc;
}

int launch_force(sph_ctx* c, bool force, bool collide, bool integrate, float dt) {
    if (c->n == 0) {
        return integrate ? advance_colliders(c, dt) : SPH_OK;
    }
    const bool mark = force_begin(c, integrate);
    int rc = launch_force_range(c, c->own_off, c->own_off + c->n, force, collide, integrate, dt, mark);
    if (rc) return rc;
    if (integrate && have_obstacle(c) && (rc = launch_obstacle_push(c, true, mark))) return rc;
    return force_finish(c, integrate, mark, dt);
}

static int launch_density_targets(sph_ctx* c, const Targets& tg, uint32_t threads) {
    if (threads == 0) return SPH_OK;
    if (c->precision == SPH_PRECISION_MIXED_F16)
        hipLaunchKernelGGL(k_density_h, dim3(ceil_div(threads, PAIR_THREADS)), dim3(PAIR_THREADS), 0, c->stream, c->posi,
                           c->keyS, c->table.cells, c->dp, c->cw, tg, c->grid, c->phys);
    else {
#define SPH_LAUNCH_DENSITY_T(T, CL)                                                                                             \
    hipLaunchKernelGGL((k_density<T, CL>), dim3(ceil_div(threads, (uint32_t)T)), dim3(T), 0, c->stream, c->posi, c->keyS,        \
                       c->table.cells, c->dp, c->cw, tg, c->grid, c->phys)
        if (pair_clamp(c)) {
            if (small_blocks(c)) SPH_LAUNCH_DENSITY_T(SMALL_THREADS_PAIR, true); else SPH_LAUNCH_DENSITY_T(DENS_THREADS, true);
        } else {
            if (small_blocks(c)) SPH_LAUNCH_DENSITY_T(SMALL_THREADS_PAIR, false); else SPH_LAUNCH_DENSITY_T(DENS_THREADS, false);
        }
#undef SPH_LAUNCH_DENSITY_T
    }
    SPH_HIP(hipGetLastError());
    return SPH_OK;
}

int launch_density_hole(sph_ctx* c, uint32_t lo, uint32_t hi, uint32_t hole_lo, uint32_t hole_hi) {
    if (hi <= lo) return SPH_OK;
    uint32_t threads;
    Targets tg = targets_with_hole(lo, hi, hole_lo, hole_hi, threads);
    tg.direct_hull = c->direct_hull;
    const uint32_t bt = c->precision == SPH_PRECISION_MIXED_F16 ? (uint32_t)PAIR_THREADS : (small_blocks(c) ? (uint32_t)SMALL_THREADS_PAIR : (uint32_t)DENS_THREADS);
    tg.order = block_order(c, ceil_div(threads, bt), c->order_ztile_dens);
    return launch_density_targets(c, tg, threads);
}

int launch_density_range(sph_ctx* c, uint32_t lo, uint32_t hi) { return launch_density_hole(c, lo, hi, hi, hi); }

int launch_density_dev_range(sph_ctx* c, const uint32_t* range_dev, uint32_t max_count) {
    const Targets tg{0u, 0u, 0xFFFFFFFFu, 0u, range_dev, c->direct_hull, BlockOrder{0u, 0u, 0u, 0u, 0u}};
    return launch_density_targets(c, tg, max_count);
}

template <class... Sph>
__global__ __launch_bounds__(256) void k_integrate(float4* __restrict__ posi, float4* __restrict__ velr,
                                                   const float2* __restrict__ dp, const float4* __restrict__ fpress,
                                                   const float4* __restrict__ fvisc, const float4* __restrict__ dvel,
                                                   float4* __restrict__ pos_by_index, uint32_t lo, uint32_t hi, float dt,
                                                   Phys ph, Sph... sp) {
    uint32_t i = lo + blockIdx.x * 256u + threadIdx.x;
    if (i >= hi) return;
    float4 pi = posi[i], vi = velr[i];
    const float4 fp = fpress[i], fv = fvisc[i], dv = dvel[i];
    integrate_one(ph, dt, pi, vi, dp[i].x, fp.x + fv.x, fp.y + fv.y, fp.z + fv.z, dv.x, dv.y, dv.z, at_slot(sp, i - lo)...);
    posi[i] = pi;
    velr[i] = vi;
    if (pos_by_index) pos_by_index[__float_as_uint(pi.w)] = make_float4(pi.x, pi.y, pi.z, 1.0f);
}

int launch_integrate(sph_ctx* c, float dt) {
    if (c->n == 0) return advance_colliders(c, dt);
    float4* const pos_out = c->slab ? nullptr : c->pos_out;
    if (c->tracked)
        hipLaunchKernelGGL(k_integrate<SpheresTracked>, dim3(ceil_div(c->n, 256)), dim3(256), 0, c->stream, c->posi, c->velr, c->dp,
                           c->fpress, c->fvisc, c->dvel, pos_out, c->own_off, c->own_off + c->n, dt, c->phys, tracked_pack(c));
    else if (c->n_colliders)
        hipLaunchKernelGGL(k_integrate<Spheres>, dim3(ceil_div(c->n, 256)), dim3(256), 0, c->stream, c->posi, c->velr, c->dp,
                           c->fpress, c->fvisc, c->dvel, pos_out, c->own_off, c->own_off + c->n, dt, c->phys, sphere_table(c));
    else
        hipLaunchKernelGGL(k_integrate<>, dim3(ceil_div(c->n, 256)), dim3(256), 0, c->stream, c->posi, c->velr, c->dp,
                           c->fpress, c->fvisc, c->dvel, pos_out, c->own_off, c->own_off + c->n, dt, c->phys);
    SPH_HIP(hipGetLastError());
    if (have_obstacle(c))
        if (int rc = launch_obstacle_push(c, false, false)) return rc;
    return advance_colliders(c, dt);
}

}
```

gpufluidsimulator_amd/csrc/sph_sort.hip:

```cpp
#include "sph_device.hpp"

#include <atomic>
#include <chrono>
#include <cstdlib>

namespace sph {

constexpr int SORT_THREADS = 256;
#ifndef SPH_SORT_KPT
#define SPH_SORT_KPT 16
#endif
constexpr int SORT_KPT = SPH_SORT_KPT;
constexpr int SORT_TILE = SORT_THREADS * SORT_KPT;

__global__ __launch_bounds__(256) void k_hash(const float4* __restrict__ posi, uint32_t n, GridDesc g,
                                              uint32_t* __restrict__ keys) {
    uint32_t i = blockIdx.x * 256u + threadIdx.x;
    if (i >= n) return;
    float4 p = posi[i];
    keys[i] = cell_key(g, p.x, p.y, p.z);
}

constexpr int OS_TILE = SORT_TILE;
constexpr uint32_t OS_DIGITS = 512;
constexpr uint32_t OS_PASSES = 4;
#ifndef SPH_OS_GROUP
#define SPH_OS_GROUP 16
#endif
constexpr uint32_t OS_GROUP = SPH_OS_GROUP;
constexpr uint32_t OS_ONE_GROUP_TILES = 64;
constexpr uint32_t OS_ALL_TILES = 0xFFFFFFFFu;
constexpr uint32_t OS_SPIN_LIMIT = 1u << 22;
#ifndef SPH_OS_PASS_GRID_MAX
#define SPH_OS_PASS_GRID_MAX 1536
#endif
constexpr uint32_t OS_PASS_GRID_MAX = SPH_OS_PASS_GRID_MAX;
#ifndef SPH_OS_PASS_THREADS
#define SPH_OS_PASS_THREADS 256
#endif
constexpr int PASS_THREADS = SPH_OS_PASS_THREADS;
constexpr int PASS_WAVES = PASS_THREADS / WAVE;
constexpr int PASS_KPT = OS_TILE / PASS_THREADS;
constexpr int PASS_WAVE_TILE = WAVE * PASS_KPT;

__device__ __forceinline__ uint32_t sort_count(uint32_t n, const uint32_t* __restrict__ n_dev) {
    return n_dev ? min(*n_dev, n) : n;
}

__device__ __forceinline__ void wave_count_digit(uint32_t* counts, uint32_t d, bool valid) {
    const uint64_t act = __ballot(valid);
    if (act == 0ull) return;
    const uint32_t d0 = (uint32_t)__builtin_amdgcn_readlane((int)d, __builtin_ctzll(act));
    if (__ballot(valid && d != d0) == 0ull) {
        if ((threadIdx.x & 63u) == (uint32_t)__builtin_ctzll(act)) atomicAdd(&counts[d0], (uint32_t)__popcll(act));
    } else if (valid) {
        atomicAdd(&counts[d], 1u);
    }
}

constexpr uint32_t OS_HIST_TILES = 2;
template <int BITS>
__global__ __launch_bounds__(SORT_THREADS) void k_os_hist(const uint32_t* __restrict__ keys, uint32_t n_arg,
                                                          const uint32_t* __restrict__ n_dev, uint32_t pass0,
                                                          uint32_t passes, uint32_t group_tiles,
                                                          uint32_t* __restrict__ hist, uint32_t small_max) {
    constexpr int RADIX = 1 << BITS;
    __shared__ uint32_t h[4 * RADIX];
    const uint32_t n = sort_count(n_arg, n_dev);
    if (n <= small_max) return;
    const uint32_t ntiles = (n + OS_TILE - 1) / OS_TILE;
    const uint32_t nchunks = (ntiles + OS_HIST_TILES - 1) / OS_HIST_TILES;
    for (uint32_t chunk = blockIdx.x; chunk < nchunks; chunk += gridDim.x) {
        for (uint32_t d = threadIdx.x; d < passes * RADIX; d += SORT_THREADS) h[d] = 0;
        __syncthreads();
        const uint32_t t0 = chunk * OS_HIST_TILES, t1 = min(t0 + OS_HIST_TILES, ntiles);
        for (uint32_t tile = t0; tile < t1; tile++) {
#pragma unroll
            for (int q = 0; q < SORT_KPT / 4; q++) {
                const uint32_t i = tile * OS_TILE + (q * SORT_THREADS + threadIdx.x) * 4u;
                uint4 k4 = make_uint4(0u, 0u, 0u, 0u);
                if (i + 3u < n) k4 = *reinterpret_cast<const uint4*>(keys + i);
                else {
                    if (i < n) k4.x = keys[i];
// ... 246 lines not shown
                        for (uint32_t q = 0; q < OS_GROUP - 1; q++) if (pending >> q & 1u) w[q] = 0;
                        break;
                    }
                    __builtin_amdgcn_s_sleep(1);
#pragma unroll
                    for (uint32_t q = 0; q < OS_GROUP - 1; q++)
                        if (pending >> q & 1u) {
                            if (DPT == 2) w[q] = __hip_atomic_load(reinterpret_cast<const os_word*>(st32 + (size_t)q * RADIX),
                                                                   __ATOMIC_RELAXED, __HIP_MEMORY_SCOPE_AGENT);
                            else w[q] = __hip_atomic_load(st32 + (size_t)q * RADIX, __ATOMIC_RELAXED, __HIP_MEMORY_SCOPE_AGENT);
                        }
#pragma unroll
                    for (uint32_t q = 0; q < OS_GROUP - 1; q++)
                        if ((pending >> q & 1u) && fresh(w[q])) pending &= ~(1u << q);
                }
#pragma unroll
                for (uint32_t q = 0; q < OS_GROUP - 1; q++)
                    if (q < npred) {
                        excl[0] += (uint32_t)w[q] & ((1u << OS_CNT_BITS) - 1u);
                        if (DPT == 2) excl[DPT - 1] += (uint32_t)(w[q] >> 32) & ((1u << OS_CNT_BITS) - 1u);
                    }
            } else if (!GROUPED && has_d && tile != gstart) {
                bool open[DPT];
#pragma unroll
                for (int k = 0; k < DPT; k++) open[k] = true;
                uint32_t spins = 0;
                for (uint32_t j = tile; j-- > gstart;) {
                    bool any_open = false;
#pragma unroll
                    for (int k = 0; k < DPT; k++) {
                        if (!open[k]) continue;
                        const os_word* src = status + (size_t)j * RADIX + threadIdx.x * DPT + k;
                        os_word w;
                        for (;;) {
                            w = __hip_atomic_load(src, __ATOMIC_RELAXED, __HIP_MEMORY_SCOPE_AGENT);
                            if ((uint32_t)(w >> 33) == epoch) break;
                            if (++spins > OS_SPIN_LIMIT) { *err = 1u; w = (os_word)1 << 32; break; }
                            __builtin_amdgcn_s_sleep(1);
                        }
                        excl[k] += (uint32_t)w;
                        if ((w >> 32) & 1ull) open[k] = false; else any_open = true;
                    }
                    if (!any_open) break;
                }
#pragma unroll
                for (int k = 0; k < DPT; k++)
                    os_publish(status + (size_t)tile * RADIX + threadIdx.x * DPT + k, epoch, true, excl[k] + cnt[k]);
            }
#pragma unroll
            for (int k = 0; k < DPT; k++) {
                const uint32_t d = threadIdx.x * DPT + k;
                if (has_d) s_delta[d] = dbase[k] + group_base[(grp * OS_PASSES) * OS_DIGITS + d] + excl[k] - tstart[k];
            }
        }
        OS_STAT(5);
        __syncthreads();
        OS_STAT(6);

        const uint32_t tile_n = min((uint32_t)OS_TILE, n - tile * OS_TILE);
#pragma unroll 4
        for (int t = 0; t < PASS_KPT; t++) {
            const uint32_t q = t * PASS_THREADS + threadIdx.x;
            if (q < tile_n) {
                const uint32_t k = s_key[q];
                const uint32_t d = (k >> shift) & (RADIX - 1);
                const uint32_t dst = s_delta[d] + q;
                kout[dst] = k;
                vout[dst] = s_val[q];
            }
        }
        OS_STAT(7);
        __syncthreads();
        OS_STAT(8);
    }
}

constexpr int SMALL_THREADS = 1024;
constexpr int SMALL_WAVES = SMALL_THREADS / WAVE;
#ifndef SPH_OS_SMALL_TILES
#define SPH_OS_SMALL_TILES 2
#endif
constexpr uint32_t OS_SMALL_MAX = SPH_OS_SMALL_TILES * OS_TILE;
constexpr int SMALL_KPT = OS_SMALL_MAX / SMALL_THREADS;
struct Front {
    uint32_t lo, cnt;
};
__device__ __forceinline__ bool mover_slot_less(uint32_t mover_slot, uint32_t slot, Front f) {
    return mover_slot < slot || mover_slot - f.lo < f.cnt;
}

__device__ __forceinline__ uint32_t mm_lower_bound(const uint32_t* __restrict__ mk, const uint32_t* __restrict__ mi, uint32_t lo, uint32_t hi,
                                                   uint32_t key, uint32_t slot, Front f) {
    return first_not(lo, hi, [&](uint32_t r) {
        const uint32_t k = mk[r];
        return k < key || (k == key && mover_slot_less(mi[r], slot, f));
    });
}

template <int BITS>
__global__ __launch_bounds__(SMALL_THREADS) void k_os_small(uint32_t* ak, uint32_t* av, uint32_t* bk, uint32_t* bv,
                                                            const uint32_t* __restrict__ n_dev, uint32_t n_cap, uint32_t passes,
                                                            bool alone, const uint32_t* __restrict__ A, uint32_t n_slots, Front front,
                                                            uint32_t* __restrict__ tileL, uint32_t* __restrict__ tileA) {
    constexpr int RADIX = 1 << BITS;
    __shared__ uint32_t s_key[OS_SMALL_MAX], s_val[OS_SMALL_MAX];
    __shared__ uint32_t wh[SMALL_WAVES][RADIX];
    __shared__ uint32_t s_wtot[SMALL_WAVES];
    const uint32_t m = min(*n_dev, n_cap);
    const uint32_t wave = threadIdx.x >> 6, lane = threadIdx.x & 63u;
    const uint64_t lt_mask = (1ull << lane) - 1ull;
    const uint32_t* kin = ak; const uint32_t* vin = av;
    uint32_t* kout = (passes & 1u) ? bk : ak; uint32_t* vout = (passes & 1u) ? bv : av;
    if (m > OS_SMALL_MAX) {
        if (!alone) return;
        uint32_t* const gbase = s_key;
        uint32_t* const ghist = s_val;
        const uint32_t wbase_t = wave * (WAVE * SMALL_KPT);
        for (uint32_t p = 0; p < passes; p++) {
            const uint32_t shift = p * BITS;
            const uint32_t* sk = (p & 1u) ? bk : ak; const uint32_t* sv = (p & 1u) ? bv : av;
            uint32_t* dk = (p & 1u) ? ak : bk; uint32_t* dv = (p & 1u) ? av : bv;
            for (int d = threadIdx.x; d < RADIX; d += SMALL_THREADS) ghist[d] = 0;
            __syncthreads();
            for (uint32_t i0 = wave * WAVE; i0 < m; i0 += SMALL_THREADS) {
                const uint32_t i = i0 + lane;
                const uint32_t k = i < m ? sk[i] : 0u;
                wave_count_digit(ghist, (k >> shift) & (RADIX - 1), i < m);
            }
            __syncthreads();
            {
                const uint32_t cnt = threadIdx.x < (uint32_t)RADIX ? ghist[threadIdx.x] : 0u;
                const uint32_t start = block_scan_excl<SMALL_WAVES>(cnt, s_wtot);
                if (threadIdx.x < (uint32_t)RADIX) gbase[threadIdx.x] = start;
            }
            __syncthreads();
            for (uint32_t tile0 = 0; tile0 < m; tile0 += OS_SMALL_MAX) {
                const uint32_t mt = min(OS_SMALL_MAX, m - tile0);
                uint32_t key[SMALL_KPT], val[SMALL_KPT];
#pragma unroll
                for (int t = 0; t < SMALL_KPT; t++) {
                    const uint32_t j = wbase_t + t * WAVE + lane;
                    key[t] = j < mt ? sk[tile0 + j] : 0xFFFFFFFFu;
                    val[t] = j < mt ? sv[tile0 + j] : 0u;
                }
                for (int d = threadIdx.x; d < SMALL_WAVES * RADIX; d += SMALL_THREADS) (&wh[0][0])[d] = 0;
                __syncthreads();
#pragma unroll
                for (int t = 0; t < SMALL_KPT; t++) {
                    if (wbase_t + t * WAVE >= mt) break;
                    wave_count_digit(wh[wave], (key[t] >> shift) & (RADIX - 1), wbase_t + t * WAVE + lane < mt);
                }
                __syncthreads();
                if (threadIdx.x < (uint32_t)RADIX) {
                    uint32_t run = gbase[threadIdx.x];
#pragma unroll
                    for (int w = 0; w < SMALL_WAVES; w++) { const uint32_t c = wh[w][threadIdx.x]; wh[w][threadIdx.x] = run; run += c; }
                    gbase[threadIdx.x] = run;
                }
                __syncthreads();
                const lds_u32_ptr pos = (lds_u32_ptr)wh[wave];
#pragma unroll
                for (int t = 0; t < SMALL_KPT; t++) {
                    if (wbase_t + t * WAVE >= mt) break;
                    const bool valid = wbase_t + t * WAVE + lane < mt;
                    const uint32_t d = (key[t] >> shift) & (RADIX - 1);
                    uint32_t dif_lo = 0u, dif_hi = 0u;
#pragma unroll
                    for (int b = 0; b < BITS; b++) {
                        const uint32_t bm = (uint32_t)__builtin_amdgcn_sbfe((int)d, b, 1);
                        const uint64_t mm = __ballot(bm != 0u);
                        dif_lo |= (uint32_t)mm ^ bm;
                        dif_hi |= (uint32_t)(mm >> 32) ^ bm;
                    }
                    const uint64_t vmask = __ballot(valid);
                    const uint32_t peers_lo = ~dif_lo & (uint32_t)vmask, peers_hi = ~dif_hi & (uint32_t)(vmask >> 32);
                    const uint32_t rank = (uint32_t)__popc(peers_lo & (uint32_t)lt_mask) + (uint32_t)__popc(peers_hi & (uint32_t)(lt_mask >> 32));
                    uint32_t base = 0;
                    if (valid) base = pos[d];
                    os_wave_lds_order();
                    if (valid && rank == 0) pos[d] = base + (uint32_t)__popc(peers_lo) + (uint32_t)__popc(peers_hi);
// ... 275 lines not shown
    if ((threadIdx.x & 63u) == 0 && (i & ~63u) < n) {
        const uint32_t chunk = i >> 6;
        mask[chunk] = m;
        if (m) atomicAdd(&tile_cnt[chunk / MM_TILE_CHUNKS], (uint32_t)__popcll(m));
    }
}

__global__ __launch_bounds__(1024) void k_mm_tilescan(uint32_t* __restrict__ tile_cnt, uint32_t nt,
                                                      uint32_t* __restrict__ tile_off, uint32_t* __restrict__ m_dev,
                                                      volatile uint32_t* __restrict__ m_host,
                                                      unsigned long long* __restrict__ m_total, uint32_t seq) {
    __shared__ uint32_t lds[1024 / 64];
    const uint32_t m = scan_array_one_block<1024>(nt, lds, [&](uint32_t t) { return tile_cnt[t]; },
                                                  [&](uint32_t t, uint32_t before) { tile_off[t] = before; tile_cnt[t] = 0; });
    if (threadIdx.x == 1023) {
        *m_dev = m; m_host[HW_MOVERS] = m;
        if (m_total) *m_total += m;
        if (seq) { __threadfence_system(); m_host[HW_COUNT_SEQ] = seq; }
    }
}

constexpr uint32_t MM_FUSED_SCAN_TILES = 2048;
__global__ __launch_bounds__(256) void k_mm_compact(const uint64_t* __restrict__ mask, uint32_t nchunks, uint32_t n_old,
                                                    const uint32_t* __restrict__ tile_off, const uint32_t* __restrict__ tile_cnt,
                                                    uint32_t nt, uint32_t* __restrict__ m_dev, volatile uint32_t* __restrict__ m_host,
                                                    unsigned long long* __restrict__ m_total,
                                                    const uint32_t* __restrict__ A, const uint32_t* __restrict__ B,
                                                    uint32_t* __restrict__ M64, uint32_t* __restrict__ mk,
                                                    uint32_t* __restrict__ mi, uint2* __restrict__ cells,
                                                    const uint32_t* __restrict__ keys_abs, uint32_t g0lo, uint32_t g0hi,
                                                    uint32_t g1lo, uint32_t g1hi) {
    if (blockIdx.x >= nt) {
        const uint32_t t = (blockIdx.x - nt) * 256u + threadIdx.x, n0 = g0hi - g0lo;
        const uint32_t lo = t < n0 ? g0lo : g1lo, hi = t < n0 ? g0hi : g1hi;
        const uint32_t s = t < n0 ? g0lo + t : g1lo + (t - n0);
        if (s >= hi) return;
        const uint32_t k = keys_abs[s];
        if (s == lo || keys_abs[s - 1] != k) cells[k] = make_uint2(0u, 0u);
        return;
    }
    __shared__ uint32_t part[256];
    uint32_t tile_start;
    if (tile_cnt) {
        uint32_t below = 0, all = 0;
        for (uint32_t t = threadIdx.x; t < nt; t += 256u) { const uint32_t v = tile_cnt[t]; all += v; below += t < blockIdx.x ? v : 0u; }
#pragma unroll
        for (int off = 32; off; off >>= 1) { below += (uint32_t)__shfl_xor((int)below, off); all += (uint32_t)__shfl_xor((int)all, off); }
        if ((threadIdx.x & 63u) == 0u) { part[threadIdx.x >> 6] = below; part[4 + (threadIdx.x >> 6)] = all; }
        __syncthreads();
        tile_start = part[0] + part[1] + part[2] + part[3];
        if (blockIdx.x == 0 && threadIdx.x == 0) {
            const uint32_t m = part[4] + part[5] + part[6] + part[7];
            *m_dev = m; m_host[HW_MOVERS] = m;
            if (m_total) *m_total += m;
        }
        __syncthreads();
    } else {
        tile_start = tile_off[blockIdx.x];
    }
    const uint32_t chunk = blockIdx.x * MM_TILE_CHUNKS + threadIdx.x;
    uint64_t m = chunk < nchunks ? mask[chunk] : 0ull;
    const uint32_t cnt = (uint32_t)__popcll(m);
    part[threadIdx.x] = cnt;
    __syncthreads();
    for (int off = 1; off < 256; off <<= 1) {
        uint32_t v = threadIdx.x >= (uint32_t)off ? part[threadIdx.x - off] : 0u;
        __syncthreads();
        part[threadIdx.x] += v;
        __syncthreads();
    }
    if (chunk >= nchunks) return;
    uint32_t at = tile_start + part[threadIdx.x] - cnt;
    M64[chunk] = at;
    while (m) {
        const uint32_t i = chunk * 64u + (uint32_t)__builtin_ctzll(m);
        m &= m - 1ull;
        mk[at] = B[i];
        mi[at] = i;
        at++;
        if (cells && i < n_old) cells[A[i]] = make_uint2(0u, 0u);
    }
}

constexpr uint32_t MM_RANK_TILE = 4096;
__global__ __launch_bounds__(256) void k_mm_tile_rank(const uint32_t* __restrict__ A, uint32_t n,
                                                      const uint32_t* __restrict__ mk, const uint32_t* __restrict__ mi,
                                                      const uint32_t* __restrict__ m_dev, uint32_t* __restrict__ tileL,
                                                      uint32_t* __restrict__ tileA, bool small_too, uint32_t small_max,
                                                      Front front) {
    const uint32_t t = blockIdx.x * 256u + threadIdx.x;
    const uint32_t ntiles = (n + MM_RANK_TILE - 1) / MM_RANK_TILE;
    if (t > ntiles) return;
    const uint32_t m = *m_dev;
    if (small_too && m <= small_max) return;
    const uint32_t slot = t * MM_RANK_TILE;
    const uint32_t a = t == ntiles ? 0xFFFFFFFFu : A[slot];
    tileA[t] = a;
    tileL[t] = t == ntiles ? m : mm_lower_bound(mk, mi, 0u, m, a, slot, front);
}

__device__ __forceinline__ void mm_scatter_body(uint32_t bid, const uint32_t* __restrict__ A, uint32_t n,
                                                const uint64_t* __restrict__ mask, const uint32_t* __restrict__ M64,
                                                const uint32_t* __restrict__ mk, const uint32_t* __restrict__ mi,
                                                const uint32_t* __restrict__ tileL, const float4* __restrict__ posi,
                                                const float4* __restrict__ velr, float4* __restrict__ posi_out,
                                                float4* __restrict__ velr_out, uint32_t* __restrict__ key_out,
                                                uint32_t* __restrict__ perm_out, Front front) {
    const uint32_t i = bid * 256u + threadIdx.x;
    const uint32_t first = __builtin_amdgcn_readfirstlane(i);
    if (first >= n) return;
    const uint32_t lane = threadIdx.x & 63u;
    const uint32_t chunk = first >> 6;
    const uint32_t last = min(first + 63u, n - 1u);
    const uint32_t tile = first / MM_RANK_TILE;
    const uint32_t b0 = tileL[tile], b1 = tileL[tile + 1];
    uint32_t L0 = b0, L1 = b0;
    if (b0 != b1) {
        L0 = mm_lower_bound(mk, mi, b0, b1, A[first], first, front);
        L1 = mm_lower_bound(mk, mi, L0, b1, A[last], last, front);
    }
    if (i >= n) return;
    const uint64_t bits = mask[chunk];
    if ((bits >> lane) & 1ull) return;
    const uint32_t key = A[i];
    const uint32_t before = M64[chunk] + (uint32_t)__popcll(bits & ((1ull << lane) - 1ull));
    const uint32_t L = L0 == L1 ? L0 : mm_lower_bound(mk, mi, L0, L1, key, i, front);
    const uint32_t dst = i - before + L;
    posi_out[dst] = posi[i];
    velr_out[dst] = velr[i];
    key_out[dst] = key;
    if (perm_out) perm_out[dst] = i;
}

__device__ __forceinline__ void mm_place_body(uint32_t bid, uint32_t nblocks, const uint32_t* __restrict__ A, uint32_t n,
                                              uint32_t nchunks, const uint64_t* __restrict__ mask,
                                              const uint32_t* __restrict__ M64, const uint32_t* __restrict__ mk,
                                              const uint32_t* __restrict__ mi, const uint32_t* __restrict__ m_dev,
                                              const uint32_t* __restrict__ tileA, const uint2* __restrict__ cells,
                                              uint32_t slot_base, const float4* __restrict__ posi,
                                              const float4* __restrict__ velr, float4* __restrict__ posi_out,
                                              float4* __restrict__ velr_out, uint32_t* __restrict__ key_out,
                                              uint32_t* __restrict__ perm_out, Front front) {
    const uint32_t m = *m_dev;
    const uint32_t ntiles = (n + MM_RANK_TILE - 1) / MM_RANK_TILE;
    for (uint32_t r = bid * 256u + threadIdx.x; r < m; r += nblocks * 256u) {
        const uint32_t key = mk[r], slot = mi[r];
        uint32_t s, e;
        uint2 ce = make_uint2(0u, 0u);
        if (cells) ce = cells[key];
        if (ce.y > ce.x) {
            s = ce.x - slot_base; e = ce.y - slot_base;
        } else {
            const uint32_t lo = first_not(0u, ntiles, [&](uint32_t t) { return tileA[t] < key; });
            s = first_not(lo ? (lo - 1u) * MM_RANK_TILE : 0u, min(lo * MM_RANK_TILE, n), [&](uint32_t i) { return A[i] < key; });
            uint32_t step = 1u, p = s;
            while (p < n && A[p] == key) { p = min(p + step, n); step <<= 1; }
            const uint32_t q = p > s ? max(s, p - (step >> 1)) : s;
            e = first_not(q, p, [&](uint32_t i) { return A[i] <= key; });
        }
        const uint32_t j = slot - front.lo < front.cnt ? s : min(max(slot, s), e);
        uint32_t before = m;
        if ((j >> 6) < nchunks) before = M64[j >> 6] + (uint32_t)__popcll(mask[j >> 6] & ((1ull << (j & 63u)) - 1ull));
        const uint32_t dst = r + (j - before);
        posi_out[dst] = posi[slot];
        velr_out[dst] = velr[slot];
        key_out[dst] = key;
        if (perm_out) perm_out[dst] = slot;
    }
}

__global__ __launch_bounds__(256) void k_mm_move(uint32_t place_blocks, uint32_t* __restrict__ zero_cnt, uint32_t zero_n,
                                                 const uint32_t* __restrict__ A, uint32_t n,
                                                 uint32_t nchunks, const uint64_t* __restrict__ mask,
                                                 const uint32_t* __restrict__ M64, const uint32_t* __restrict__ mk,
                                                 const uint32_t* __restrict__ mi, const uint32_t* __restrict__ m_dev,
                                                 const uint32_t* __restrict__ tileL, const uint32_t* __restrict__ tileA,
                                                 const uint2* __restrict__ cells, uint32_t slot_base,
                                                 const float4* __restrict__ posi, const float4* __restrict__ velr,
                                                 float4* __restrict__ posi_out, float4* __restrict__ velr_out,
                                                 uint32_t* __restrict__ key_out, uint32_t* __restrict__ perm_out, Front front) {
    if (zero_cnt && blockIdx.x * 256u + threadIdx.x < zero_n) zero_cnt[blockIdx.x * 256u + threadIdx.x] = 0u;
    if (blockIdx.x < place_blocks)
        mm_place_body(blockIdx.x, place_blocks, A, n, nchunks, mask, M64, mk, mi, m_dev, tileA, cells, slot_base, posi, velr,
                      posi_out, velr_out, key_out, perm_out, front);
    else
        mm_scatter_body(blockIdx.x - place_blocks, A, n, mask, M64, mk, mi, tileL, posi, velr, posi_out, velr_out, key_out,
                        perm_out, front);
}

static uint32_t merge_grid_for(uint32_t movers_hint, uint32_t n) {
    const uint32_t want = max(ceil_div(2u * movers_hint + 1u, SORT_TILE) + 15u, OS_ONE_GROUP_TILES);
    return min(want, max(ceil_div(n, SORT_TILE), 1u));
}

static void mm_tilescan(sph_ctx* c, uint32_t n, bool counted) {
    const uint32_t nt = ceil_div(ceil_div(n, 64u), MM_TILE_CHUNKS);
    uint32_t seq = 0u;
    if (counted) { if (++c->marks.scan_seq == 0u) c->marks.scan_seq = 1u; seq = c->marks.scan_seq; }
    hipLaunchKernelGGL(k_mm_tilescan, dim3(1), dim3(1024), 0, c->stream, c->mm_tile_cnt, nt, c->mm_tile_off, c->mm_count,
                       c->mm_count_host_dev, counted ? c->mm_total : (unsigned long long*)nullptr, seq);
    c->marks.counted_valid = counted;
}

static uint32_t mm_tiles(uint32_t n) { return ceil_div(ceil_div(n, 64u), MM_TILE_CHUNKS); }

static void launch_mm_mark(sph_ctx* c, uint32_t n) {
    hipLaunchKernelGGL(k_mm_mark, dim3(ceil_div(n, 256)), dim3(256), 0, c->stream, c->keyS + c->own_off, c->k0, n, c->mm_mask,
                       c->mm_tile_cnt);
}

void mm_set_marks(sph_ctx* c) {
    c->marks.marked = true; c->marks.scanned = false; c->marks.off = c->own_off; c->marks.n = c->n;
}

void mm_scan_marks(sph_ctx* c) {
    if (!c->marks.marked || c->marks.scanned) return;
    if (c->mm_count_host[HW_MOVERS] != 0u && mm_tiles(c->marks.n) <= MM_FUSED_SCAN_TILES) return;
    mm_tilescan(c, c->marks.n, true);
    c->marks.scanned = true;
}

void mm_drop_marks(sph_ctx* c, bool counted) {
    if (!c->marks.marked) return;
    if (!c->marks.scanned) mm_tilescan(c, c->marks.n, counted);
    c->marks.marked = false;
    c->marks.scanned = false;
}

static bool launch_merge_count(sph_ctx* c, uint32_t n) {
    if (c->marks.marked && !(c->marks.off == c->own_off && c->marks.n == n)) mm_drop_marks(c);
    if (!c->marks.marked) {
        launch_mm_mark(c, n);
        c->marks.scanned = false;
    }
    bool in_compact = false;
    if (!c->marks.scanned) {
        if (mm_tiles(n) <= MM_FUSED_SCAN_TILES) { in_compact = true; c->marks.counted_valid = false; }
        else mm_tilescan(c, n, true);
    }
    c->marks.marked = false;
    c->marks.scanned = false;
    return in_compact;
}

static bool mm_counted_none(const sph_ctx* c) {
    volatile const uint32_t* hw = c->mm_count_host;
    return c->marks.counted_valid && hw[HW_COUNT_SEQ] == c->marks.scan_seq && (std::atomic_thread_fence(std::memory_order_acquire), hw[HW_MOVERS] == 0u);
}

__global__ __launch_bounds__(256) void k_mm_mark_tail(uint32_t n_old, uint32_t n_tot, uint64_t* __restrict__ mask,
                                                      uint32_t* __restrict__ tile_cnt) {
    const uint32_t chunk = blockIdx.x * 256u + threadIdx.x;
    if (chunk * 64u >= n_tot) return;
    const uint32_t lo = chunk * 64u, hi = min(lo + 64u, n_tot);
    uint64_t m = 0ull;
    if (hi > n_old) {
        const uint32_t first = max(lo, n_old) - lo, cnt = hi - lo;
        m = (cnt == 64u ? ~0ull : ((1ull << cnt) - 1ull)) & ~((1ull << first) - 1ull);
        atomicAdd(&tile_cnt[chunk / MM_TILE_CHUNKS], (uint32_t)__popcll(m));
    }
    mask[chunk] = m;
}

static int launch_sort_merge(sph_ctx* c, uint32_t n, uint32_t n_tot, bool table_live, uint32_t hint, Front front = Front{0u, 0u},
                             bool count_in_compact = false, bool clear_ghosts = false) {
    const uint32_t* A = c->keyS + c->own_off;
    const uint32_t* B = c->k0;
    const uint32_t nchunks = ceil_div(n_tot, 64u), nt = ceil_div(nchunks, MM_TILE_CHUNKS);
    uint32_t* mk = c->mm_k0; uint32_t* mi = c->v0; uint32_t* mk2 = c->mm_k1; uint32_t* mi2 = c->mm_v1;
    const uint32_t gc[4] = {clear_ghosts ? c->table.lo : 0u, clear_ghosts ? c->own_off : 0u, clear_ghosts ? c->own_off + n : 0u,
                            clear_ghosts ? c->table.hi : 0u};
    const uint32_t gc_blocks = ceil_div((gc[1] - gc[0]) + (gc[3] - gc[2]), 256u);
    hipLaunchKernelGGL(k_mm_compact, dim3(nt + gc_blocks), dim3(256), 0, c->stream, c->mm_mask, nchunks, n, c->mm_tile_off,
                       count_in_compact ? c->mm_tile_cnt : (const uint32_t*)nullptr, nt, c->mm_count, c->mm_count_host_dev, c->mm_total, A, B,
                       c->mm_M64, mk, mi, table_live ? c->table.cells : (uint2*)nullptr, c->keyS, gc[0], gc[1], gc[2], gc[3]);
    SPH_HIP(hipGetLastError());
    SmallTail tail;
    int form = SORT_FORM_BOTH;
    tail.A = A; tail.n_slots = n; tail.front = front; tail.hint = hint; tail.form = &form;
    int rc = radix_sort_pairs(c, n_tot, c->mm_count, merge_grid_for(hint, n_tot), false, mk, mi, mk2, mi2, tail);
    if (rc) return rc;
    if (form != SORT_FORM_SMALL) {
        const uint32_t rank_tiles = ceil_div(n, MM_RANK_TILE) + 1u;
        hipLaunchKernelGGL(k_mm_tile_rank, dim3(ceil_div(rank_tiles, 256u)), dim3(256), 0, c->stream, A, n, mk, mi, c->mm_count,
                           c->mm_tileL, c->mm_tileA, form == SORT_FORM_BOTH, OS_SMALL_MAX, front);
        SPH_HIP(hipGetLastError());
    }
    uint32_t* perm = c->keep_perm ? c->v1 : (uint32_t*)nullptr;
    const float4* ps = c->posi + c->own_off; const float4* vs = c->velr + c->own_off;
    float4* po = c->posi2 + c->gcap; float4* vo = c->velr2 + c->gcap; uint32_t* ko = c->keyS2 + c->gcap;
    const uint32_t place_blocks = min(max(ceil_div(2u * hint + 1u, 256u) + 15u, 512u), 65535u);
    hipLaunchKernelGGL(k_mm_move, dim3(place_blocks + ceil_div(n, 256)), dim3(256), 0, c->stream, place_blocks,
                       count_in_compact ? c->mm_tile_cnt : (uint32_t*)nullptr, nt, A, n, nchunks,
                       c->mm_mask, c->mm_M64, mk, mi, c->mm_count, c->mm_tileL, c->mm_tileA,
                       table_live ? c->table.cells : (const uint2*)nullptr, c->own_off, ps, vs, po, vo, ko, perm, front);
    SPH_HIP(hipGetLastError());
    c->last_perm = perm;
    return SPH_OK;
}

static int sort_throttle(sph_ctx* c) {
    volatile const uint32_t* hw = c->mm_count_host;
    if ((int32_t)(c->sort_seq_issued - hw[HW_BUILD_SEQ]) < 4) return SPH_OK;
    const auto t0 = std::chrono::steady_clock::now();
    for (uint32_t spins = 1; (int32_t)(c->sort_seq_issued - hw[HW_BUILD_SEQ]) >= 4; spins++) {
        __builtin_ia32_pause();
        if ((spins & 0xFFFu) == 0u) {
            const hipError_t q = hipStreamQuery(c->stream);
            if (q == hipSuccess) break;
            if (q != hipErrorNotReady) SPH_HIP(q);
            SPH_REQUIRE(std::chrono::duration<double>(std::chrono::steady_clock::now() - t0).count() < 300.0, SPH_E_DEVICE,
                        "sort: the device has not reached the table build of sort %u after 300 s", c->sort_seq_issued - 3u);
        }
    }
    return SPH_OK;
}

static bool sort_skip_if_still(sph_ctx* c, bool was_still, TableLeft left, bool count_in_compact, int* rc) {
    if (!(was_still && left != TableLeft::NOTHING && c->own_off == c->gcap && !count_in_compact && mm_counted_none(c))) return false;
    c->sort_merges++;
    c->sort_skips++;
    c->last_sort_skipped = true;
    c->last_perm = nullptr;
    c->order_valid = true;
    *rc = left == TableLeft::OWNED_AND_GHOSTS ? table_drop_ghosts(c) : SPH_OK;
    return true;
}

static int sort_by_merge(sph_ctx* c, uint32_t n, TableLeft left, bool count_in_compact) {
    const bool table_live = left != TableLeft::NOTHING;
    int rc = launch_sort_merge(c, n, n, table_live, c->mm_count_host[HW_MOVERS], Front{0u, 0u}, count_in_compact,
                               left == TableLeft::OWNED_AND_GHOSTS);
    if (rc) return rc;
    c->sort_merges++;
    if (c->table.valid && !table_live) rc = launch_cells_clear(c);
    return rc;
}

static int sort_full(sph_ctx* c, uint32_t n, bool can_merge) {
    if (c->table.valid) {
        int rc = launch_cells_clear(c);
        if (rc) return rc;
    }
    if (c->marks.marked) {
        mm_drop_marks(c, true);
    } else if (can_merge && (c->sort_calls & 7u) == 0) {
        launch_mm_mark(c, n);
        mm_tilescan(c, n, true);
        SPH_HIP(hipGetLastError());
    }
    uint32_t* kin = c->k0; uint32_t* vin = c->v0;
    uint32_t* kout = c->k1; uint32_t* vout = c->v1;
    int rc = radix_sort_pairs(c, n, nullptr, ceil_div(n, SORT_TILE), true, kin, vin, kout, vout);
    if (rc) return rc;
    hipLaunchKernelGGL(k_reorder, dim3(ceil_div(n, 256)), dim3(256), 0, c->stream, kin, vin, n, c->posi + c->own_off,
                       c->velr + c->own_off, c->posi2 + c->gcap, c->velr2 + c->gcap, c->keyS2 + c->gcap);
    SPH_HIP(hipGetLastError());
    c->last_perm = vin;
    return SPH_OK;
}

static int sort_finish(sph_ctx* c, uint32_t n, bool* owned_build_pending) {
    swap_state(c, true);
    table_forget(c);
    if (++c->sort_seq_issued == 0u) c->sort_seq_issued = 1u;
    if (owned_build_pending) {
        *owned_build_pending = true;
    } else {
        int rc = launch_cells_build_range(c, c->gcap, c->gcap + n, c->sort_seq_issued);
        if (rc) return rc;
    }
    c->order_valid = true;
    table_set(c, c->gcap, c->gcap + n);
    return SPH_OK;
}

int launch_sort(sph_ctx* c, bool* owned_build_pending) {
    if (owned_build_pending) *owned_build_pending = false;
    const uint32_t n = c->n;
    if (n == 0) return SPH_OK;
    const uint32_t nblocks = ceil_div(n, SORT_TILE);
    SPH_REQUIRE(nblocks <= c->sort_blocks_cap, SPH_E_CAPACITY, "sort: %u blocks > capacity %u", nblocks,
                c->sort_blocks_cap);
    if (c->sort_merge && !c->host_paced) { const int rc = sort_throttle(c); if (rc) return rc; }
    c->sort_calls++;
    c->last_sort_skipped = false;
    const bool can_merge = c->sort_merge && c->order_valid;
    const TableLeft left = table_take_left(c);
    int rc;
    if (can_merge && (c->mm_count_host[HW_MOVERS] <= n / 8u || c->sort_merge_always)) {
        const bool was_still = c->mm_count_host[HW_MOVERS] == 0u;
        const bool count_in_compact = launch_merge_count(c, n);
        if (sort_skip_if_still(c, was_still, left, count_in_compact, &rc)) return rc;
        rc = sort_by_merge(c, n, left, count_in_compact);
    } else {
        rc = sort_full(c, n, can_merge);
    }
    if (rc) return rc;
    return sort_finish(c, n, owned_build_pending);
}

int launch_merge_arrivals(sph_ctx* c, uint32_t n_in, uint32_t n_front) {
    const uint32_t n = c->n, n_tot = n + n_in;
    SPH_REQUIRE(c->order_valid && table_covers(c, c->own_off, c->own_off + n), SPH_E_STATE,
                "launch_merge_arrivals needs the sorted owned range and its cell table");
    SPH_REQUIRE(ceil_div(n_tot, SORT_TILE) <= c->sort_blocks_cap, SPH_E_CAPACITY, "sort: capacity exceeded");
    mm_drop_marks(c);
    const uint32_t nchunks = ceil_div(n_tot, 64u);
    hipLaunchKernelGGL(k_mm_mark_tail, dim3(ceil_div(nchunks, 256u)), dim3(256), 0, c->stream, n, n_tot, c->mm_mask,
                       c->mm_tile_cnt);
    mm_tilescan(c, n_tot, false);
    SPH_HIP(hipGetLastError());
    int rc = launch_sort_merge(c, n, n_tot, true, n_in, Front{n, n_front < n_in ? n_front : n_in});
    if (rc) return rc;
    swap_state(c, true);
    c->n = n_tot;
    table_forget(c);
    rc = launch_cells_build_range(c, c->gcap, c->gcap + n_tot);
    if (rc) return rc;
    table_set(c, c->gcap, c->gcap + n_tot);
    c->order_valid = true;
    c->keys_fresh = false;
    c->n_glo = c->n_ghi = 0;
    c->stage = sph_ctx::ST_SORTED;
    results_stale(c);
    return SPH_OK;
}

const uint32_t* last_sort_permutation(sph_ctx* c) { return c->last_perm; }

int sort_indices_by_key(sph_ctx* c, const uint32_t* keys_dev, uint32_t n, uint32_t bits, const uint32_t** perm_out) {
    *perm_out = nullptr;
    if (n == 0) return SPH_OK;
    const uint32_t nblocks = ceil_div(n, SORT_TILE);
    SPH_REQUIRE(nblocks <= c->sort_blocks_cap && n <= c->cap, SPH_E_CAPACITY, "sort: %u keys > capacity %u", n, c->cap);
    SPH_HIP(hipMemcpyAsync(c->k0, keys_dev, (size_t)n * sizeof(uint32_t), hipMemcpyDeviceToDevice, c->stream));
    uint32_t* kin = c->k0; uint32_t* vin = c->v0;
    uint32_t* kout = c->k1; uint32_t* vout = c->v1;
    const uint32_t saved = c->key_bits;
    c->key_bits = bits;
    const int rc = radix_sort_pairs(c, n, nullptr, nblocks, true, kin, vin, kout, vout);
    c->key_bits = saved;
    if (rc) return rc;
    c->keys_fresh = false;
    c->last_perm = nullptr;
    *perm_out = vin;
    return SPH_OK;
}

int sort_buffers_alloc(sph_ctx* c) {
    Buffers& m = c->mem;
    const size_t cap = c->cap;
    c->sort_blocks_cap = ceil_div(c->cap, (uint32_t)OS_TILE) + 1;
    const size_t tiles = c->sort_blocks_cap, groups = tiles / 4 + 3;
    c->os_groups_cap = (uint32_t)groups;
    static_assert(MM_RANK_TILE >= (uint32_t)OS_TILE, "mm_tileL / mm_tileA: an entry per MM_RANK_TILE slots + the end fit into one per sort tile + 2");
    int rc = m.alloc(&c->k0, cap, false);
    if (!rc) rc = m.alloc(&c->v0, cap, false);
    if (!rc) rc = m.alloc(&c->k1, cap, false);
    if (!rc) rc = m.alloc(&c->v1, cap, false);
    if (!rc) rc = m.alloc(&c->os_hist, groups * OS_PASSES * OS_DIGITS, true);
    if (!rc) rc = m.alloc(&c->os_base, groups * OS_PASSES * OS_DIGITS, false);
    if (!rc) rc = m.alloc(&c->os_tickets, (size_t)OS_PASSES * groups, true);
    if (!rc) rc = m.alloc(&c->os_tot, (size_t)OS_PASSES * OS_DIGITS, false);
    if (!rc) rc = m.alloc(&c->os_status, (size_t)OS_DIGITS * tiles, true);
    if (!rc) rc = m.alloc(&c->os_status32, (size_t)OS_DIGITS * tiles, true);
    if (!rc) rc = m.alloc(&c->mm_tileL, tiles + 2, false);
    if (!rc) rc = m.alloc(&c->mm_tileA, tiles + 2, false);
    if (!rc) rc = m.alloc_host(&c->os_err_host, 1, &c->os_err_dev);
    if (!rc) *c->os_err_host = 0;
    if (!rc) rc = m.alloc(&c->d_scratch, (size_t)SCRATCH_WORDS, false);
    if (!rc) rc = m.alloc_host(&c->h_scratch, (size_t)SCRATCH_WORDS);
    const char* env = getenv("SPH_SORT_MERGE");
    c->sort_merge = !(env && env[0] == '0');
    const size_t nchunks = (size_t)ceil_div(c->cap, 64u) + 1, ntiles = nchunks / MM_TILE_CHUNKS + 2;
    if (!rc) rc = m.alloc(&c->mm_mask, nchunks, false);
    if (!rc) rc = m.alloc(&c->mm_M64, nchunks, false);
// ... 17 lines not shown
```

include/sph_hip.h:

```cpp
#ifndef SPH_HIP_H
#define SPH_HIP_H

#include <stddef.h>
#include <stdint.h>

#ifdef __cplusplus
extern "C" {
#endif

#define SPH_ABI_VERSION 2

enum {
    SPH_OK = 0,
    SPH_E_INVALID = -1,
    SPH_E_DEVICE = -2,
    SPH_E_NOMEM = -3,
    SPH_E_CAPACITY = -4,
    SPH_E_STATE = -5,
    SPH_E_PEER = -6
};

typedef struct sph_ctx sph_ctx;

typedef struct sph_params {
// ... 129 lines not shown
    float rot[9];
    float trans[3];
    float focal_px;
    float near_z, far_z;
} sph_camera;
enum { SPH_COLOR_INDEX = 0, SPH_COLOR_SPEED = 1, SPH_COLOR_DENSITY = 2 };
typedef struct sph_render_style {
    int32_t  color_mode;
    float    lo, hi;
    float    radius;
    uint32_t index_count;
    uint8_t  background[4];
} sph_render_style;
int sph_camera_look_at(sph_camera* out, uint32_t width, uint32_t height, const float eye[3], const float target[3],
                       const float up[3], float fovy_deg, float near_z, float far_z);
int sph_render(sph_ctx* c, const sph_camera* camera, const sph_render_style* style);
int sph_render_read(sph_ctx* c, uint8_t* rgba, uint32_t* id, float* depth);
int sph_render_image_dev(sph_ctx* c, void** rgba_dev, uint32_t* width, uint32_t* height);

#define SPH_SURFACE_MAX_RADIUS_PX 16
#define SPH_SURFACE_MAX_ITERATIONS 8
typedef struct sph_surface_style {
    uint32_t smooth_radius_px;
    uint32_t smooth_iterations;
    float    depth_falloff;
    int32_t  flat_color;
    float    tint[3];
    float    absorb[3];
    float    light[3];
    float    specular;
} sph_surface_style;
void sph_surface_defaults(sph_surface_style* s);
int sph_render_surface(sph_ctx* c, const sph_camera* camera, const sph_render_style* style, const sph_surface_style* surface);
int sph_render_surface_read(sph_ctx* c, float* raw_depth, uint32_t* thickness_q, float* normal_xyz);

#define SPH_MESH_MAX_REACH 8
#define SPH_MESH_MAX_DIM 2048
#define SPH_MESH_MAX_NODES (1u << 27)
typedef struct sph_mesh_params {
    float spacing;
    float radius;
    float iso;
} sph_mesh_params;
void sph_mesh_defaults(sph_mesh_params* p);
int sph_mesh_lattice(const sph_ctx* c, const sph_mesh_params* p, uint32_t dims[3], float origin[3]);
int sph_mesh_extract(sph_ctx* c, const sph_mesh_params* p, uint32_t* n_vertices, uint32_t* n_triangles);
int sph_mesh_read(sph_ctx* c, float* pos_xyz, float* normal_xyz, uint32_t* tri);
int sph_mesh_dev(sph_ctx* c, void** pos_dev, void** normal_dev, void** tri_dev, uint32_t* n_vertices, uint32_t* n_triangles);
int sph_mesh_save_obj(sph_ctx* c, const char* path);
 int sph_mesh_field_dims(sph_ctx* c, uint32_t dims[3]);
 int sph_mesh_field_read(sph_ctx* c, uint32_t* counts);

int sph_snapshot_save(sph_ctx* c, const char* path);
int sph_snapshot_load(sph_ctx* c, const char* path);
int sph_snapshot_info(const char* path, uint32_t* n, sph_params* p);

 int sph_get_keys(sph_ctx* c, uint32_t* keys);
 int sph_get_order(sph_ctx* c, uint32_t* index);
 int sph_get_cell_range(sph_ctx* c, uint32_t cell, uint32_t* start, uint32_t* end);
 int sph_get_cells(sph_ctx* c, uint32_t max_cells, uint32_t* key, uint32_t* start, uint32_t* count);
 uint32_t sph_cell_key(const sph_ctx* c, uint32_t x, uint32_t y, uint32_t z);

int sph_hash(sph_ctx* c);
int sph_sort(sph_ctx* c);
int sph_build_cells(sph_ctx* c);
int sph_density(sph_ctx* c);
int sph_force(sph_ctx* c);
int sph_collide(sph_ctx* c);
int sph_integrate(sph_ctx* c, float dt);
int sph_step(sph_ctx* c, float dt, uint32_t n_steps);
int sph_step_phased(sph_ctx* c, float dt, uint32_t n_steps);
int sph_force_collide_integrate(sph_ctx* c, float dt);

int sph_timing_enable(sph_ctx* c, int on);
int sph_timing_get(sph_ctx* c, float ms[SPH_PH_COUNT], uint32_t* n_steps);
int sph_timing_reset(sph_ctx* c);
 int sph_sort_stats(sph_ctx* c, uint64_t* sorts, uint64_t* merges, uint64_t* skips, uint32_t* last_movers,
                   uint64_t* movers_total);
 int sph_sort_forms(const sph_ctx* c, uint64_t out[3]);
 int sph_set_sort_mode(sph_ctx* c, int merge);
 int sph_set_direct_hull(sph_ctx* c, uint32_t slots);
 int sph_set_pair_small_launch(sph_ctx* c, uint32_t slots);
 int sph_set_block_order(sph_ctx* c, int xcd, int ztile, uint32_t strip_blocks_log2);
 int sph_last_sort_skipped(const sph_ctx* c);

#define SPH_HALO_RECORD_FLOATS 8
int sph_migrants_count(sph_ctx* c, uint32_t count[2]);
int sph_slab_counts(sph_ctx* c, uint32_t count[4]);
int sph_migrants_pack(sph_ctx* c, void* buf_dev[2], uint32_t capacity);
int sph_migrants_append(sph_ctx* c, const void* buf_dev, uint32_t n);
int sph_halo_count(sph_ctx* c, uint32_t count[2]);
int sph_halo_pack(sph_ctx* c, void* buf_dev[2], uint32_t capacity);
int sph_halo_pack_counts(sph_ctx* c, void* buf_dev[2], uint32_t capacity, const uint32_t count[2]);
int sph_halo_unpack(sph_ctx* c, const void* lo_dev, uint32_t n_lo, const void* hi_dev, uint32_t n_hi);
int sph_halo_pack_density(sph_ctx* c, void* buf_dev[2], uint32_t capacity);
int sph_halo_unpack_density(sph_ctx* c, const void* lo_dev, const void* hi_dev);
int sph_layer_histogram(sph_ctx* c, uint32_t* hist, uint32_t n_layers);

enum { SPH_TAG_MIGRANTS = 1, SPH_TAG_HALO_A = 2, SPH_TAG_HALO_B = 3, SPH_TAG_MIGRANTS_REST = 4, SPH_TAG_PING = 5,
       SPH_TAG_RECUT_COUNTS = 6, SPH_TAG_RECUT = 7,
       SPH_TAG_ONE = 8,
       SPH_TAG_ONE_REST = 9 };
typedef struct sph_transport {
    void* self;
    int (*exchange)(void* self, int tag, const void* send_lo, size_t send_lo_bytes, void* recv_lo, size_t recv_lo_bytes,
                    const void* send_hi, size_t send_hi_bytes, void* recv_hi, size_t recv_hi_bytes, void* hip_stream);
    int host_buffers;
    void (*abort)(void* self);
} sph_transport;

int sph_rccl_unique_id(uint8_t id[128]);
int sph_rccl_transport_create(sph_transport** out, const uint8_t id[128], int rank, int world, int device);
void sph_rccl_transport_destroy(sph_transport* t);
 int sph_rccl_transport_selftest(sph_transport* t, size_t bytes);
 int sph_rccl_transport_info(const sph_transport* t, int out[4]);

typedef struct sph_local_hub sph_local_hub;
int sph_local_hub_create(sph_local_hub** out, int world, int device);
void sph_local_hub_destroy(sph_local_hub* hub);
int sph_local_hub_set_timeout(sph_local_hub* hub, double seconds);
int sph_local_transport_create(sph_transport** out, sph_local_hub* hub, int rank);
void sph_local_transport_destroy(sph_transport* t);

 int sph_loop_transport_create(sph_transport** out, float z_shift, double link_gbs, double latency_us);
 void sph_loop_transport_destroy(sph_transport* t);

typedef struct sph_slab sph_slab;
int sph_slab_create(sph_slab** out, sph_ctx* ctx, int rank, int world, const sph_transport* transport,
                    uint32_t migrant_capacity);
void sph_slab_destroy(sph_slab* s);
int sph_slab_step(sph_slab* s, float dt, uint32_t n_steps);
int sph_slab_sync(sph_slab* s);
int sph_slab_set_wait_timeout(sph_slab* s, double seconds);
 int sph_slab_stats(const sph_slab* s, uint64_t out[5]);
 int sph_slab_counters(const sph_slab* s, uint64_t out[8]);
 uint64_t sph_slab_in_place_merges(const sph_slab* s);
 uint64_t sph_slab_exchanges(const sph_slab* s);
int sph_slab_recut(sph_slab* s, uint32_t new_z_lo, uint32_t new_z_hi);
 int sph_slab_recut_stats(const sph_slab* s, uint64_t out[2]);
int sph_slab_ping(sph_slab* s, size_t bytes, uint32_t reps, double out[3]);
enum {
    SPH_SLAB_T_STEPS = 0, SPH_SLAB_T_WAITS_READY = 1,
    SPH_SLAB_T_WAIT = 2,
    SPH_SLAB_T_PRE = 4, SPH_SLAB_T_POST = 6, SPH_SLAB_T_HOST = 8,
    SPH_SLAB_T_GROUPS = 10,
    SPH_SLAB_T_GROUPS_ONE = 22,
    SPH_SLAB_T_WORDS = 28
};
int sph_slab_timing_enable(sph_slab* s, int on);
int sph_slab_timing_reset(sph_slab* s);
int sph_slab_timing_get(sph_slab* s, double out[SPH_SLAB_T_WORDS]);
 int sph_slab_set_early_force(sph_slab* s, int on);
int sph_slab_set_protocol(sph_slab* s, int groups);
 int sph_slab_protocol(const sph_slab* s, uint64_t out[3]);
 int sph_slab_early_force_stats(const sph_slab* s, uint64_t out[2]);
 int sph_test_trust_mover_hint(sph_ctx* c);
 int sph_slab_test_raise_flag(sph_slab* s, int flag);
 void sph_memory_stats(uint64_t out[3]);
 void sph_test_fail_alloc(uint32_t k);
 int sph_test_scan(sph_ctx* c, int bits, uint32_t n, const void* in, void* out, void* total);
 int sph_test_lower_bounds(sph_ctx* c, const uint32_t* keys, uint32_t n, const uint32_t* targets, uint32_t m, uint32_t* out);
 void sph_test_guard(uint32_t band_bytes, int fill_unzeroed);
 int sph_test_guard_check(uint64_t out[4]);
int sph_slab_failed(const sph_slab* s);

#ifdef __cplusplus
// ... 4 lines not shown
```

Measured before the change: 4.607 billion particle-steps/s.

## Split velocity scatter out of merge sort and overlap it with density kernel

During merge-based sorting, only positions, keys and the permutation are moved. The velocity scatter is deferred: spare blocks inside the density kernel perform it, reusing stored destinations and chunk brackets, or a separate kernel flushes it before the force pass. This takes velocity traffic off the sort's critical path and hides it behind density work, which does not read velocities. Density occupancy is also raised from 6 to 7. The cost is extra bracket and destination storage, added complexity, and possible interference with density blocks.

New measurement: 4.658 billion particle-steps/s, median of 4. About the same (+1.1%).

```diff
diff --git a/gpufluidsimulator_amd/capi.py b/gpufluidsimulator_amd/capi.py
--- a/gpufluidsimulator_amd/capi.py
+++ b/gpufluidsimulator_amd/capi.py
@@ -236,6 +236,8 @@
     "sph_set_pair_small_launch": (C.c_int, [_P, C.c_uint32]),
     "sph_set_block_order": (C.c_int, [_P, C.c_int, C.c_int, C.c_uint32]),
     "sph_sort_forms": (C.c_int, [_P, C.POINTER(C.c_uint64)]),
+    "sph_set_move_split": (C.c_int, [_P, C.c_int]),
+    "sph_move_split_stats": (C.c_int, [_P, C.POINTER(C.c_uint64)]),
     "sph_test_trust_mover_hint": (C.c_int, [_P]),
     "sph_memory_stats": (None, [C.POINTER(C.c_uint64)]),
     "sph_test_fail_alloc": (None, [C.c_uint32]),
@@ -825,6 +827,14 @@
         _check(self.L.sph_sort_forms(self.h, out))
         return tuple(int(v) for v in out)
 
+    def set_move_split(self, on=1):
+        _check(self.L.sph_set_move_split(self.h, int(on)))
+
+    def move_split_stats(self):
+        out = (C.c_uint64 * 2)()
+        _check(self.L.sph_move_split_stats(self.h, out))
+        return tuple(int(v) for v in out)
+
     def set_block_order(self, xcd=True, ztile=True, strip_blocks_log2=4):
         _check(self.L.sph_set_block_order(self.h, int(bool(xcd)), int(bool(ztile)), int(strip_blocks_log2)))
 
diff --git a/gpufluidsimulator_amd/csrc/sph_capi.hip b/gpufluidsimulator_amd/csrc/sph_capi.hip
--- a/gpufluidsimulator_amd/csrc/sph_capi.hip
+++ b/gpufluidsimulator_amd/csrc/sph_capi.hip
@@ -277,6 +277,10 @@
         int v = 1;
         if (sscanf(env, "%d", &v) == 1) c->pair_clamp = v != 0;
     }
+    if (const char* env = getenv("SPH_MOVE_SPLIT")) {
+        int v = 1;
+        if (sscanf(env, "%d", &v) == 1) c->move_split = v >= 0 && v <= 3 ? v : 1;
+    }
     if (rc) { m.free_all(); delete c; return rc; }
     *out = c;
     return SPH_OK;
@@ -308,9 +312,9 @@
     return SPH_OK;
 }
 
-int step_sort(sph_ctx* c, bool* owned_build_pending) {
+int step_sort(sph_ctx* c, bool* owned_build_pending, bool split_vel) {
     PhaseTimer t(c, SPH_PH_SORT);
-    int rc = launch_sort(c, owned_build_pending);
+    int rc = launch_sort(c, owned_build_pending, split_vel);
     if (rc) return rc;
     c->n_glo = c->n_ghi = 0;
     c->halo_n_valid = false;
@@ -1019,9 +1023,10 @@
     SPH_HIP(hipSetDevice(c->device));
     for (uint32_t s = 0; s < n_steps; s++) {
         int rc = step_hash(c);
-        if (!rc) rc = step_sort(c);
+        if (!rc) rc = step_sort(c, nullptr, true);
         if (!rc) rc = step_cells(c);
         if (!rc) rc = do_density(c);
+        if (c->vel_move.pending) { const int frc = flush_vel_move(c); if (!rc) rc = frc; }
         if (rc) return rc;
         {
             PhaseTimer t(c, SPH_PH_FORCE);
@@ -1137,6 +1142,19 @@
     return SPH_OK;
 }
 
+int sph_set_move_split(sph_ctx* c, int on) {
+    SPH_REQUIRE(c, SPH_E_INVALID, "null context");
+    SPH_REQUIRE(on >= 0 && on <= 3, SPH_E_INVALID, "move split %d: 0 to 3", on);
+    c->move_split = on;
+    return SPH_OK;
+}
+
+int sph_move_split_stats(const sph_ctx* c, uint64_t out[2]) {
+    SPH_REQUIRE(c && out, SPH_E_INVALID, "null argument");
+    out[0] = c->move_splits; out[1] = c->move_flushes;
+    return SPH_OK;
+}
+
 int sph_sort_stats(sph_ctx* c, uint64_t* sorts, uint64_t* merges, uint64_t* skips, uint32_t* last_movers,
                    uint64_t* movers_total) {
     SPH_REQUIRE(c, SPH_E_INVALID, "null context");
diff --git a/gpufluidsimulator_amd/csrc/sph_common.hpp b/gpufluidsimulator_amd/csrc/sph_common.hpp
--- a/gpufluidsimulator_amd/csrc/sph_common.hpp
+++ b/gpufluidsimulator_amd/csrc/sph_common.hpp
@@ -169,6 +169,28 @@
     uint32_t off = 0, n = 0;
     uint32_t scan_seq = 0;
     bool counted_valid = false;
+};
+
+struct VelMove {
+    const uint32_t* A;
+    const uint64_t* mask;
+    const uint32_t* M64;
+    const uint32_t* mk;
+    const uint32_t* mi;
+    const uint32_t* mdst;
+    const uint32_t* m_dev;
+    const uint32_t* tileL;
+    const uint2* bracket;
+    const uint32_t* tileA;
+    const float4* velr;
+    float4* velr_out;
+    uint32_t n, nchunks;
+    uint32_t blocks;
+    uint32_t period;
+};
+struct PendingVelMove {
+    VelMove args{};
+    bool pending = false;
 };
 
 enum HostWord : uint32_t {
@@ -307,6 +329,9 @@
     sph::MoverMarks marks;
     uint32_t* mm_tileL = nullptr;
     uint32_t* mm_tileA = nullptr;
+    int move_split = 1;
+    sph::PendingVelMove vel_move;
+    uint64_t move_splits = 0, move_flushes = 0;
     uint32_t* d_scratch = nullptr;
     uint32_t* h_scratch = nullptr;
 
@@ -343,7 +368,8 @@
 int launch_hash(sph_ctx* c);
 int launch_reset_lattice(sph_ctx* c, const uint32_t lattice[3], int jitter, const float jitter_dims[3], uint64_t start,
                          uint32_t count);
-int launch_sort(sph_ctx* c, bool* owned_build_pending = nullptr);
+int launch_sort(sph_ctx* c, bool* owned_build_pending = nullptr, bool split_vel = false);
+int flush_vel_move(sph_ctx* c);
 int launch_merge_arrivals(sph_ctx* c, uint32_t n_in, uint32_t n_front = 0);
 int launch_cells_clear(sph_ctx* c);
 void table_forget(sph_ctx* c);
@@ -371,7 +397,7 @@
 int force_finish(sph_ctx* c, bool integrate, bool mark, float dt);
 int set_slab_range(sph_ctx* c, uint32_t z_lo, uint32_t z_hi);
 int step_hash(sph_ctx* c, bool ghosts_to_sort = false);
-int step_sort(sph_ctx* c, bool* owned_build_pending = nullptr);
+int step_sort(sph_ctx* c, bool* owned_build_pending = nullptr, bool split_vel = false);
 int step_cells(sph_ctx* c);
 int launch_integrate(sph_ctx* c, float dt);
 inline bool have_obstacle(const sph_ctx* c) { return c->ob_phi != nullptr; }
diff --git a/gpufluidsimulator_amd/csrc/sph_move.hpp b/gpufluidsimulator_amd/csrc/sph_move.hpp
--- /dev/null
+++ b/gpufluidsimulator_amd/csrc/sph_move.hpp
@@ -0,0 +1,157 @@
+#pragma once
+
+#include "sph_device.hpp"
+
+namespace sph {
+
+struct Front {
+    uint32_t lo, cnt;
+};
+__device__ __forceinline__ bool mover_slot_less(uint32_t mover_slot, uint32_t slot, Front f) {
+    return mover_slot < slot || mover_slot - f.lo < f.cnt;
+}
+
+__device__ __forceinline__ uint32_t mm_lower_bound(const uint32_t* __restrict__ mk, const uint32_t* __restrict__ mi, uint32_t lo, uint32_t hi,
+                                                   uint32_t key, uint32_t slot, Front f) {
+    return first_not(lo, hi, [&](uint32_t r) {
+        const uint32_t k = mk[r];
+        return k < key || (k == key && mover_slot_less(mi[r], slot, f));
+    });
+}
+
+constexpr uint32_t MM_RANK_TILE = 4096;
+
+__device__ __forceinline__ bool mm_scatter_dst(uint32_t i, const uint32_t* __restrict__ A, uint32_t n,
+                                               const uint64_t* __restrict__ mask, const uint32_t* __restrict__ M64,
+                                               const uint32_t* __restrict__ mk, const uint32_t* __restrict__ mi,
+                                               const uint32_t* __restrict__ tileL, const uint2* __restrict__ bracket_in,
+                                               uint2* __restrict__ bracket_out, Front front, bool need_key, uint32_t& key,
+                                               uint32_t& dst) {
+    const uint32_t first = __builtin_amdgcn_readfirstlane(i);
+    if (first >= n) return false;
+    const uint32_t lane = threadIdx.x & 63u;
+    const uint32_t chunk = first >> 6;
+    uint32_t L0, L1;
+    if (bracket_in) {
+        const uint2 br = bracket_in[chunk];
+        L0 = __builtin_amdgcn_readfirstlane(br.x); L1 = __builtin_amdgcn_readfirstlane(br.y);
+    } else {
+        const uint32_t last = min(first + 63u, n - 1u);
+        const uint32_t tile = first / MM_RANK_TILE;
+        const uint32_t b0 = tileL[tile], b1 = tileL[tile + 1];
+        L0 = b0; L1 = b0;
+        if (b0 != b1) {
+            L0 = mm_lower_bound(mk, mi, b0, b1, A[first], first, front);
+            L1 = mm_lower_bound(mk, mi, L0, b1, A[last], last, front);
+        }
+        if (bracket_out && lane == 0u) bracket_out[chunk] = make_uint2(L0, L1);
+    }
+    if (i >= n) return false;
+    const uint64_t bits = mask[chunk];
+    if ((bits >> lane) & 1ull) return false;
+    const uint32_t before = M64[chunk] + (uint32_t)__popcll(bits & ((1ull << lane) - 1ull));
+    key = 0u;
+    if (need_key || L0 != L1) key = A[i];
+    const uint32_t L = L0 == L1 ? L0 : mm_lower_bound(mk, mi, L0, L1, key, i, front);
+    dst = i - before + L;
+    return true;
+}
+
+template <bool POS, bool VEL>
+__device__ __forceinline__ void mm_scatter_body(uint32_t i, const uint32_t* __restrict__ A, uint32_t n,
+                                                const uint64_t* __restrict__ mask, const uint32_t* __restrict__ M64,
+                                                const uint32_t* __restrict__ mk, const uint32_t* __restrict__ mi,
+                                                const uint32_t* __restrict__ tileL, const float4* __restrict__ posi,
+                                                const float4* __restrict__ velr, float4* __restrict__ posi_out,
+                                                float4* __restrict__ velr_out, uint32_t* __restrict__ key_out,
+                                                uint32_t* __restrict__ perm_out, uint2* __restrict__ bracket_out, Front front) {
+    uint32_t key, dst;
+    if (!mm_scatter_dst(i, A, n, mask, M64, mk, mi, tileL, nullptr, bracket_out, front, POS, key, dst)) return;
+    if (POS) {
+        posi_out[dst] = posi[i];
+        key_out[dst] = key;
+        if (perm_out) perm_out[dst] = i;
+    }
+    if (VEL) velr_out[dst] = velr[i];
+}
+
+template <bool POS, bool VEL>
+__device__ __forceinline__ void mm_place_body(uint32_t bid, uint32_t nblocks, uint32_t threads, const uint32_t* __restrict__ A, uint32_t n,
+                                              uint32_t nchunks, const uint64_t* __restrict__ mask,
+                                              const uint32_t* __restrict__ M64, const uint32_t* __restrict__ mk,
+                                              const uint32_t* __restrict__ mi, const uint32_t* __restrict__ m_dev,
+                                              const uint32_t* __restrict__ tileA, const uint2* __restrict__ cells,
+                                              uint32_t slot_base, const float4* __restrict__ posi,
+                                              const float4* __restrict__ velr, float4* __restrict__ posi_out,
+                                              float4* __restrict__ velr_out, uint32_t* __restrict__ key_out,
+                                              uint32_t* __restrict__ perm_out, uint32_t* __restrict__ mdst, Front front) {
+    const uint32_t m = *m_dev;
+    const uint32_t ntiles = (n + MM_RANK_TILE - 1) / MM_RANK_TILE;
+    for (uint32_t r = bid * threads + threadIdx.x; r < m; r += nblocks * threads) {
+        const uint32_t slot = mi[r];
+        uint32_t key = 0u, dst;
+        if (!POS && mdst) {
+            dst = mdst[r];
+        } else {
+            key = mk[r];
+            uint32_t s, e;
+            uint2 ce = make_uint2(0u, 0u);
+            if (cells) ce = cells[key];
+            if (ce.y > ce.x) {
+                s = ce.x - slot_base; e = ce.y - slot_base;
+            } else {
+                const uint32_t lo = first_not(0u, ntiles, [&](uint32_t t) { return tileA[t] < key; });
+                s = first_not(lo ? (lo - 1u) * MM_RANK_TILE : 0u, min(lo * MM_RANK_TILE, n), [&](uint32_t i) { return A[i] < key; });
+                uint32_t step = 1u, p = s;
+                while (p < n && A[p] == key) { p = min(p + step, n); step <<= 1; }
+                const uint32_t q = p > s ? max(s, p - (step >> 1)) : s;
+                e = first_not(q, p, [&](uint32_t i) { return A[i] <= key; });
+            }
+            const uint32_t j = slot - front.lo < front.cnt ? s : min(max(slot, s), e);
+            uint32_t before = m;
+            if ((j >> 6) < nchunks) before = M64[j >> 6] + (uint32_t)__popcll(mask[j >> 6] & ((1ull << (j & 63u)) - 1ull));
+            dst = r + (j - before);
+        }
+        if (POS) {
+            posi_out[dst] = posi[slot];
+            key_out[dst] = key;
+            if (perm_out) perm_out[dst] = slot;
+            if (!VEL && mdst) mdst[r] = dst;
+        }
+        if (VEL) velr_out[dst] = velr[slot];
+    }
+}
+
+__device__ __forceinline__ bool spare_block(uint32_t b, uint32_t blocks, uint32_t period, uint32_t& idx) {
+    const uint32_t r = b >> 3, k = r / period, rounds = blocks >> 3;
+    if (r == k * period && k < rounds) { idx = k * 8u + (b & 7u); return true; }
+    idx = b - 8u * min(rounds, k + 1u);
+    return false;
+}
+constexpr uint32_t VEL_SHARE = 4096;
+inline uint32_t vel_move_blocks(uint32_t n) { return ((n + VEL_SHARE - 1u) / VEL_SHARE + 7u) & ~7u; }
+
+constexpr uint32_t VEL_BATCH = 4;
+template <int THREADS>
+__device__ __forceinline__ void vel_move_block(const VelMove& vm, uint32_t sb) {
+    static_assert(THREADS % 64 == 0 && VEL_SHARE % (VEL_BATCH * THREADS) == 0, "whole waves, whole batches of a share");
+    mm_place_body<false, true>(sb, vm.blocks, (uint32_t)THREADS, vm.A, vm.n, vm.nchunks, vm.mask, vm.M64, vm.mk, vm.mi, vm.m_dev, vm.tileA,
+                               nullptr, 0u, nullptr, vm.velr, nullptr, vm.velr_out, nullptr, nullptr, const_cast<uint32_t*>(vm.mdst),
+                               Front{0u, 0u});
+    if (sb * VEL_SHARE >= vm.n) return;
+    const uint32_t lo = sb * VEL_SHARE + threadIdx.x;
+    static_assert(VEL_BATCH == 4, "the batch is written out");
+    auto load = [&](uint32_t i) { return vm.velr[min(i, vm.n - 1u)]; };
+    auto store = [&](uint32_t i, const float4& v) {
+        uint32_t key, dst;
+        if (mm_scatter_dst(i, vm.A, vm.n, vm.mask, vm.M64, vm.mk, vm.mi, vm.tileL, vm.bracket, nullptr, Front{0u, 0u}, false, key, dst))
+            vm.velr_out[dst] = v;
+    };
+    for (uint32_t s = 0; s < VEL_SHARE; s += VEL_BATCH * (uint32_t)THREADS) {
+        const uint32_t i0 = lo + s, i1 = i0 + (uint32_t)THREADS, i2 = i1 + (uint32_t)THREADS, i3 = i2 + (uint32_t)THREADS;
+        const float4 v0 = load(i0), v1 = load(i1), v2 = load(i2), v3 = load(i3);
+        store(i0, v0); store(i1, v1); store(i2, v2); store(i3, v3);
+    }
+}
+
+}
diff --git a/gpufluidsimulator_amd/csrc/sph_pairs.hip b/gpufluidsimulator_amd/csrc/sph_pairs.hip
--- a/gpufluidsimulator_amd/csrc/sph_pairs.hip
+++ b/gpufluidsimulator_amd/csrc/sph_pairs.hip
@@ -1,4 +1,5 @@
 #include "sph_device.hpp"
+#include "sph_move.hpp"
 
 namespace sph {
 
@@ -211,7 +212,7 @@
 }
 
 #ifndef SPH_DENS_OCC
-#define SPH_DENS_OCC 6
+#define SPH_DENS_OCC 7
 #endif
 #ifndef SPH_FORCE_OCC
 #define SPH_FORCE_OCC 5
@@ -323,20 +324,25 @@
     BlockOrder order;
 };
 
-__device__ __forceinline__ uint32_t pair_block() {
-    const uint32_t rot = max(gridDim.x >> 6, 1u);
-    return blockIdx.x < rot ? gridDim.x - rot + blockIdx.x : blockIdx.x - rot;
-}
-
-__device__ __forceinline__ bool wave_targets(const Targets& T, uint32_t wave, uint32_t lane, uint32_t& i, uint32_t& hi,
-                                             uint32_t& first) {
+__device__ __forceinline__ uint32_t pair_block(uint32_t b, uint32_t nb) {
+    const uint32_t rot = max(nb >> 6, 1u);
+    return b < rot ? nb - rot + b : b - rot;
+}
+__device__ __forceinline__ uint32_t pair_block() { return pair_block(blockIdx.x, gridDim.x); }
+
+__device__ __forceinline__ bool wave_targets(const Targets& T, uint32_t b, uint32_t nb, uint32_t wave, uint32_t lane, uint32_t& i,
+                                             uint32_t& hi, uint32_t& first) {
     uint32_t lo = T.lo;
     hi = T.hi;
     if (T.dev) { lo = T.dev[0]; hi = T.dev[1]; }
-    first = lo + (ordered_block(pair_block(), gridDim.x, T.order) * (blockDim.x >> 6) + wave) * WAVE;
+    first = lo + (ordered_block(pair_block(b, nb), nb, T.order) * (blockDim.x >> 6) + wave) * WAVE;
     if (first >= T.gap_lo) first += T.gap_len;
     i = first + lane;
     return first < hi;
+}
+__device__ __forceinline__ bool wave_targets(const Targets& T, uint32_t wave, uint32_t lane, uint32_t& i, uint32_t& hi,
+                                             uint32_t& first) {
+    return wave_targets(T, blockIdx.x, gridDim.x, wave, lane, i, hi, first);
 }
 
 #ifdef SPH_PAIR_STATS
@@ -359,14 +365,17 @@
                                                                    const uint32_t* __restrict__ keyS,
                                                                    const uint2* __restrict__ cells,
                                                                    float2* __restrict__ dp, float2* __restrict__ cw,
-                                                                   Targets tg, GridDesc g, Phys ph) {
+                                                                   Targets tg, GridDesc g, Phys ph, VelMove vm) {
+    uint32_t blk;
+    if (spare_block(blockIdx.x, vm.blocks, vm.period, blk)) { vel_move_block<THREADS>(vm, blk); return; }
+    const uint32_t nblk = gridDim.x - vm.blocks;
     static_assert(UNROLL % 2 == 0, "the z-pair walk reads candidates two at a time");
     constexpr int DENS_ENT = lds_ent(THREADS);
     __shared__ float2 s_xy[DENS_ENT];
     __shared__ __attribute__((aligned(8))) float s_z[DENS_ENT];
     __shared__ __attribute__((aligned(8))) float s_zo_[DENS_ENT + 2];
     float* const s_zo = s_zo_ + 2;
-    if (tg.dev && tg.dev[0] + ordered_block(pair_block(), gridDim.x, tg.order) * (uint32_t)THREADS >= tg.dev[1]) return;
+    if (tg.dev && tg.dev[0] + ordered_block(pair_block(blk, nblk), nblk, tg.order) * (uint32_t)THREADS >= tg.dev[1]) return;
     for (uint32_t k = threadIdx.x; k < DENS_ENT; k += THREADS) {
         s_xy[k] = make_float2(0.f, 0.f);
         s_z[k] = 0.f;
@@ -377,7 +386,7 @@
     const uint32_t wave = threadIdx.x >> 6, lane = threadIdx.x & 63u;
     const uint32_t slice = wave * PIECE;
     uint32_t i, tgt_hi, wave_first;
-    if (!wave_targets(tg, wave, lane, i, tgt_hi, wave_first)) return;
+    if (!wave_targets(tg, blk, nblk, wave, lane, i, tgt_hi, wave_first)) return;
     const bool active = i < tgt_hi;
     const uint32_t ii = active ? i : tgt_hi - 1;
     const float4 pi = posi[ii];
@@ -1283,15 +1292,24 @@
         hipLaunchKernelGGL(k_density_h, dim3(ceil_div(threads, PAIR_THREADS)), dim3(PAIR_THREADS), 0, c->stream, c->posi,
                            c->keyS, c->table.cells, c->dp, c->cw, tg, c->grid, c->phys);
     else {
+        VelMove vm{};
+        const bool take_move = c->vel_move.pending && !tg.dev && c->move_split != 3;
+        if (take_move) vm = c->vel_move.args;
 #define SPH_LAUNCH_DENSITY_T(T, CL)                                                                                             \
-    hipLaunchKernelGGL((k_density<T, CL>), dim3(ceil_div(threads, (uint32_t)T)), dim3(T), 0, c->stream, c->posi, c->keyS,        \
-                       c->table.cells, c->dp, c->cw, tg, c->grid, c->phys)
+    do {                                                                                                                        \
+        const uint32_t nd = ceil_div(threads, (uint32_t)T);                                                                     \
+        vm.period = vm.blocks ? nd / vm.blocks + 1u : 1u;                                                                       \
+        hipLaunchKernelGGL((k_density<T, CL>), dim3(nd + vm.blocks), dim3(T), 0, c->stream, c->posi, c->keyS, c->table.cells,    \
+                           c->dp, c->cw, tg, c->grid, c->phys, vm);                                                             \
+    } while (0)
         if (pair_clamp(c)) {
             if (small_blocks(c)) SPH_LAUNCH_DENSITY_T(SMALL_THREADS_PAIR, true); else SPH_LAUNCH_DENSITY_T(DENS_THREADS, true);
         } else {
             if (small_blocks(c)) SPH_LAUNCH_DENSITY_T(SMALL_THREADS_PAIR, false); else SPH_LAUNCH_DENSITY_T(DENS_THREADS, false);
         }
 #undef SPH_LAUNCH_DENSITY_T
+        SPH_HIP(hipGetLastError());
+        if (take_move) c->vel_move.pending = false;
     }
     SPH_HIP(hipGetLastError());
     return SPH_OK;
diff --git a/gpufluidsimulator_amd/csrc/sph_sort.hip b/gpufluidsimulator_amd/csrc/sph_sort.hip
--- a/gpufluidsimulator_amd/csrc/sph_sort.hip
+++ b/gpufluidsimulator_amd/csrc/sph_sort.hip
@@ -1,4 +1,5 @@
 #include "sph_device.hpp"
+#include "sph_move.hpp"
 
 #include <atomic>
 #include <chrono>
@@ -411,20 +412,6 @@
 #endif
 constexpr uint32_t OS_SMALL_MAX = SPH_OS_SMALL_TILES * OS_TILE;
 constexpr int SMALL_KPT = OS_SMALL_MAX / SMALL_THREADS;
-struct Front {
-    uint32_t lo, cnt;
-};
-__device__ __forceinline__ bool mover_slot_less(uint32_t mover_slot, uint32_t slot, Front f) {
-    return mover_slot < slot || mover_slot - f.lo < f.cnt;
-}
-
-__device__ __forceinline__ uint32_t mm_lower_bound(const uint32_t* __restrict__ mk, const uint32_t* __restrict__ mi, uint32_t lo, uint32_t hi,
-                                                   uint32_t key, uint32_t slot, Front f) {
-    return first_not(lo, hi, [&](uint32_t r) {
-        const uint32_t k = mk[r];
-        return k < key || (k == key && mover_slot_less(mi[r], slot, f));
-    });
-}
 
 template <int BITS>
 __global__ __launch_bounds__(SMALL_THREADS) void k_os_small(uint32_t* ak, uint32_t* av, uint32_t* bk, uint32_t* bv,
@@ -866,7 +853,6 @@
     }
 }
 
-constexpr uint32_t MM_RANK_TILE = 4096;
 __global__ __launch_bounds__(256) void k_mm_tile_rank(const uint32_t* __restrict__ A, uint32_t n,
                                                       const uint32_t* __restrict__ mk, const uint32_t* __restrict__ mi,
                                                       const uint32_t* __restrict__ m_dev, uint32_t* __restrict__ tileL,
@@ -883,76 +869,7 @@
     tileL[t] = t == ntiles ? m : mm_lower_bound(mk, mi, 0u, m, a, slot, front);
 }
 
-__device__ __forceinline__ void mm_scatter_body(uint32_t bid, const uint32_t* __restrict__ A, uint32_t n,
-                                                const uint64_t* __restrict__ mask, const uint32_t* __restrict__ M64,
-                                                const uint32_t* __restrict__ mk, const uint32_t* __restrict__ mi,
-                                                const uint32_t* __restrict__ tileL, const float4* __restrict__ posi,
-                                                const float4* __restrict__ velr, float4* __restrict__ posi_out,
-                                                float4* __restrict__ velr_out, uint32_t* __restrict__ key_out,
-                                                uint32_t* __restrict__ perm_out, Front front) {
-    const uint32_t i = bid * 256u + threadIdx.x;
-    const uint32_t first = __builtin_amdgcn_readfirstlane(i);
-    if (first >= n) return;
-    const uint32_t lane = threadIdx.x & 63u;
-    const uint32_t chunk = first >> 6;
-    const uint32_t last = min(first + 63u, n - 1u);
-    const uint32_t tile = first / MM_RANK_TILE;
-    const uint32_t b0 = tileL[tile], b1 = tileL[tile + 1];
-    uint32_t L0 = b0, L1 = b0;
-    if (b0 != b1) {
-        L0 = mm_lower_bound(mk, mi, b0, b1, A[first], first, front);
-        L1 = mm_lower_bound(mk, mi, L0, b1, A[last], last, front);
-    }
-    if (i >= n) return;
-    const uint64_t bits = mask[chunk];
-    if ((bits >> lane) & 1ull) return;
-    const uint32_t key = A[i];
-    const uint32_t before = M64[chunk] + (uint32_t)__popcll(bits & ((1ull << lane) - 1ull));
-    const uint32_t L = L0 == L1 ? L0 : mm_lower_bound(mk, mi, L0, L1, key, i, front);
-    const uint32_t dst = i - before + L;
-    posi_out[dst] = posi[i];
-    velr_out[dst] = velr[i];
-    key_out[dst] = key;
-    if (perm_out) perm_out[dst] = i;
-}
-
-__device__ __forceinline__ void mm_place_body(uint32_t bid, uint32_t nblocks, const uint32_t* __restrict__ A, uint32_t n,
-                                              uint32_t nchunks, const uint64_t* __restrict__ mask,
-                                              const uint32_t* __restrict__ M64, const uint32_t* __restrict__ mk,
-                                              const uint32_t* __restrict__ mi, const uint32_t* __restrict__ m_dev,
-                                              const uint32_t* __restrict__ tileA, const uint2* __restrict__ cells,
-                                              uint32_t slot_base, const float4* __restrict__ posi,
-                                              const float4* __restrict__ velr, float4* __restrict__ posi_out,
-                                              float4* __restrict__ velr_out, uint32_t* __restrict__ key_out,
-                                              uint32_t* __restrict__ perm_out, Front front) {
-    const uint32_t m = *m_dev;
-    const uint32_t ntiles = (n + MM_RANK_TILE - 1) / MM_RANK_TILE;
-    for (uint32_t r = bid * 256u + threadIdx.x; r < m; r += nblocks * 256u) {
-        const uint32_t key = mk[r], slot = mi[r];
-        uint32_t s, e;
-        uint2 ce = make_uint2(0u, 0u);
-        if (cells) ce = cells[key];
-        if (ce.y > ce.x) {
-            s = ce.x - slot_base; e = ce.y - slot_base;
-        } else {
-            const uint32_t lo = first_not(0u, ntiles, [&](uint32_t t) { return tileA[t] < key; });
-            s = first_not(lo ? (lo - 1u) * MM_RANK_TILE : 0u, min(lo * MM_RANK_TILE, n), [&](uint32_t i) { return A[i] < key; });
-            uint32_t step = 1u, p = s;
-            while (p < n && A[p] == key) { p = min(p + step, n); step <<= 1; }
-            const uint32_t q = p > s ? max(s, p - (step >> 1)) : s;
-            e = first_not(q, p, [&](uint32_t i) { return A[i] <= key; });
-        }
-        const uint32_t j = slot - front.lo < front.cnt ? s : min(max(slot, s), e);
-        uint32_t before = m;
-        if ((j >> 6) < nchunks) before = M64[j >> 6] + (uint32_t)__popcll(mask[j >> 6] & ((1ull << (j & 63u)) - 1ull));
-        const uint32_t dst = r + (j - before);
-        posi_out[dst] = posi[slot];
-        velr_out[dst] = velr[slot];
-        key_out[dst] = key;
-        if (perm_out) perm_out[dst] = slot;
-    }
-}
-
+template <bool VEL>
 __global__ __launch_bounds__(256) void k_mm_move(uint32_t place_blocks, uint32_t* __restrict__ zero_cnt, uint32_t zero_n,
                                                  const uint32_t* __restrict__ A, uint32_t n,
                                                  uint32_t nchunks, const uint64_t* __restrict__ mask,
@@ -962,15 +879,18 @@
                                                  const uint2* __restrict__ cells, uint32_t slot_base,
                                                  const float4* __restrict__ posi, const float4* __restrict__ velr,
                                                  float4* __restrict__ posi_out, float4* __restrict__ velr_out,
-                                                 uint32_t* __restrict__ key_out, uint32_t* __restrict__ perm_out, Front front) {
+                                                 uint32_t* __restrict__ key_out, uint32_t* __restrict__ perm_out,
+                                                 uint32_t* __restrict__ mdst, uint2* __restrict__ bracket, Front front) {
     if (zero_cnt && blockIdx.x * 256u + threadIdx.x < zero_n) zero_cnt[blockIdx.x * 256u + threadIdx.x] = 0u;
     if (blockIdx.x < place_blocks)
-        mm_place_body(blockIdx.x, place_blocks, A, n, nchunks, mask, M64, mk, mi, m_dev, tileA, cells, slot_base, posi, velr,
-                      posi_out, velr_out, key_out, perm_out, front);
+        mm_place_body<true, VEL>(blockIdx.x, place_blocks, 256u, A, n, nchunks, mask, M64, mk, mi, m_dev, tileA, cells, slot_base, posi,
+                                 velr, posi_out, velr_out, key_out, perm_out, mdst, front);
     else
-        mm_scatter_body(blockIdx.x - place_blocks, A, n, mask, M64, mk, mi, tileL, posi, velr, posi_out, velr_out, key_out,
-                        perm_out, front);
-}
+        mm_scatter_body<true, VEL>((blockIdx.x - place_blocks) * 256u + threadIdx.x, A, n, mask, M64, mk, mi, tileL, posi, velr, posi_out,
+                                   velr_out, key_out, perm_out, bracket, front);
+}
+
+__global__ __launch_bounds__(256) void k_mm_move_vel(VelMove vm) { vel_move_block<256>(vm, blockIdx.x); }
 
 static uint32_t merge_grid_for(uint32_t movers_hint, uint32_t n) {
     const uint32_t want = max(ceil_div(2u * movers_hint + 1u, SORT_TILE) + 15u, OS_ONE_GROUP_TILES);
@@ -1047,7 +967,7 @@
 }
 
 static int launch_sort_merge(sph_ctx* c, uint32_t n, uint32_t n_tot, bool table_live, uint32_t hint, Front front = Front{0u, 0u},
-                             bool count_in_compact = false, bool clear_ghosts = false) {
+                             bool count_in_compact = false, bool clear_ghosts = false, bool split_vel = false) {
     const uint32_t* A = c->keyS + c->own_off;
     const uint32_t* B = c->k0;
     const uint32_t nchunks = ceil_div(n_tot, 64u), nt = ceil_div(nchunks, MM_TILE_CHUNKS);
@@ -1074,11 +994,24 @@
     const float4* ps = c->posi + c->own_off; const float4* vs = c->velr + c->own_off;
     float4* po = c->posi2 + c->gcap; float4* vo = c->velr2 + c->gcap; uint32_t* ko = c->keyS2 + c->gcap;
     const uint32_t place_blocks = min(max(ceil_div(2u * hint + 1u, 256u) + 15u, 512u), 65535u);
-    hipLaunchKernelGGL(k_mm_move, dim3(place_blocks + ceil_div(n, 256)), dim3(256), 0, c->stream, place_blocks,
-                       count_in_compact ? c->mm_tile_cnt : (uint32_t*)nullptr, nt, A, n, nchunks,
-                       c->mm_mask, c->mm_M64, mk, mi, c->mm_count, c->mm_tileL, c->mm_tileA,
-                       table_live ? c->table.cells : (const uint2*)nullptr, c->own_off, ps, vs, po, vo, ko, perm, front);
+    const bool stored = split_vel && c->move_split != 2 && 2u * nchunks <= c->cap;
+    uint32_t* const mdst = stored ? c->k1 : (uint32_t*)nullptr;
+    uint2* const bracket = stored ? reinterpret_cast<uint2*>(mk2) : (uint2*)nullptr;
+#define SPH_LAUNCH_MM_MOVE(VEL)                                                                                                 \
+    hipLaunchKernelGGL(k_mm_move<VEL>, dim3(place_blocks + ceil_div(n, 256)), dim3(256), 0, c->stream, place_blocks,             \
+                       count_in_compact ? c->mm_tile_cnt : (uint32_t*)nullptr, nt, A, n, nchunks,                                \
+                       c->mm_mask, c->mm_M64, mk, mi, c->mm_count, c->mm_tileL, c->mm_tileA,                                     \
+                       table_live ? c->table.cells : (const uint2*)nullptr, c->own_off, ps, vs, po, vo, ko, perm, mdst, bracket,   \
+                       front)
+    if (split_vel) SPH_LAUNCH_MM_MOVE(false); else SPH_LAUNCH_MM_MOVE(true);
+#undef SPH_LAUNCH_MM_MOVE
     SPH_HIP(hipGetLastError());
+    if (split_vel) {
+        c->vel_move.args = VelMove{A, c->mm_mask, c->mm_M64, mk, mi, mdst, c->mm_count, c->mm_tileL, bracket, c->mm_tileA, vs, vo, n, nchunks,
+                                   vel_move_blocks(n), 1u};
+        c->vel_move.pending = true;
+        c->move_splits++;
+    }
     c->last_perm = perm;
     return SPH_OK;
 }
@@ -1111,10 +1044,10 @@
     return true;
 }
 
-static int sort_by_merge(sph_ctx* c, uint32_t n, TableLeft left, bool count_in_compact) {
+static int sort_by_merge(sph_ctx* c, uint32_t n, TableLeft left, bool count_in_compact, bool split_vel) {
     const bool table_live = left != TableLeft::NOTHING;
     int rc = launch_sort_merge(c, n, n, table_live, c->mm_count_host[HW_MOVERS], Front{0u, 0u}, count_in_compact,
-                               left == TableLeft::OWNED_AND_GHOSTS);
+                               left == TableLeft::OWNED_AND_GHOSTS, split_vel);
     if (rc) return rc;
     c->sort_merges++;
     if (c->table.valid && !table_live) rc = launch_cells_clear(c);
@@ -1159,7 +1092,16 @@
     return SPH_OK;
 }
 
-int launch_sort(sph_ctx* c, bool* owned_build_pending) {
+int flush_vel_move(sph_ctx* c) {
+    if (!c->vel_move.pending) return SPH_OK;
+    c->vel_move.pending = false;
+    c->move_flushes++;
+    hipLaunchKernelGGL(k_mm_move_vel, dim3(c->vel_move.args.blocks), dim3(256), 0, c->stream, c->vel_move.args);
+    SPH_HIP(hipGetLastError());
+    return SPH_OK;
+}
+
+int launch_sort(sph_ctx* c, bool* owned_build_pending, bool split_vel) {
     if (owned_build_pending) *owned_build_pending = false;
     const uint32_t n = c->n;
     if (n == 0) return SPH_OK;
@@ -1176,7 +1118,8 @@
         const bool was_still = c->mm_count_host[HW_MOVERS] == 0u;
         const bool count_in_compact = launch_merge_count(c, n);
         if (sort_skip_if_still(c, was_still, left, count_in_compact, &rc)) return rc;
-        rc = sort_by_merge(c, n, left, count_in_compact);
+        rc = sort_by_merge(c, n, left, count_in_compact,
+                           split_vel && c->move_split && !c->slab && !owned_build_pending && c->precision == SPH_PRECISION_F32);
     } else {
         rc = sort_full(c, n, can_merge);
     }
diff --git a/include/sph_hip.h b/include/sph_hip.h
--- a/include/sph_hip.h
+++ b/include/sph_hip.h
@@ -235,6 +235,8 @@
  int sph_set_direct_hull(sph_ctx* c, uint32_t slots);
  int sph_set_pair_small_launch(sph_ctx* c, uint32_t slots);
  int sph_set_block_order(sph_ctx* c, int xcd, int ztile, uint32_t strip_blocks_log2);
+ int sph_set_move_split(sph_ctx* c, int on);
+ int sph_move_split_stats(const sph_ctx* c, uint64_t out[2]);
  int sph_last_sort_skipped(const sph_ctx* c);
 
 #define SPH_HALO_RECORD_FLOATS 8
```
